# nauful/NLZM

Measured on AMD Instinct MI355X. Metric: compress MB/s, higher is better.
Workload: dtype u8; 1 GPU; enwik9 stand-in: 1000000000 B stream, -window:28; step = 41 launches of 8 chunks (40136704 B) of the stream; timed: bytes [200683520, 401367040) of 1000000000 (a prefix: the steps asked for end before the stream does); window_bits=28, batch_chunks=8, whole_stream=False

## Files before the change

nlzm_amd/csrc/nlzm_kernels.hip:

```cpp
#include <hip/hip_runtime.h>
#include <type_traits>
#include <cstddef>
#include <stdint.h>

#include "nlzm_core.h"
#include "nlzm_v2.h"

namespace nlzm {

#ifndef NLZM_LPW
#define NLZM_LPW 64
#endif
#ifndef NLZM_AHEAD
#define NLZM_AHEAD 3
#endif
constexpr uint32_t kAhead = NLZM_AHEAD;
constexpr uint32_t kEntryWords = 16;
union V2Lds {
    v2::FLds f; v2::TLds t; v2::PLds p;
    uint32_t wq[512 * kAhead * kEntryWords];
};
__shared__ V2Lds g_v2_lds;
}
namespace xw {
// ... 51 lines not shown
    for (int k = 0; k < 4; k++) {
        const uint32_t o = threadIdx.x + 256u * k;
        const unsigned long long a = blk0 + o;
        if (a >= a1) continue;
        uint32_t h = 0, h2 = 0;
        const bool ok = a + kPfLen <= n;
        if (ok) {
#pragma unroll 13
            for (uint32_t j = 0; j < kPfLen; j++) { h = (h + tile[o + j]) * 0x2F0FD693u; h2 = (h2 ^ tile[o + j]) * 0x01000193u + 0x7F4A7C15u; }
        }
        hbuf[a - a0] = h; hbuf2[a - a0] = h2;
        uint8_t f = 0;
        if (ok) {
            const unsigned long long sl = pf_slot(h, h2, t_bits);
            if (t_bitmap) f = (T[sl >> 5] >> (sl & 31u)) & 1u;
            else { const uint32_t t = T[sl]; f = t != 0 && (uint32_t)a - (t - 1) <= wmask; }
            atomicMin(&M[(h * kPfMul2) >> (32 - m_bits)], (uint32_t)a);
        }
        c1[a - a0] = f;
    }
}

__global__ __launch_bounds__(256) void prefilter_mark_kernel(unsigned long long n, uint32_t a0, uint32_t a1, uint32_t m_bits,
                                                             const uint32_t *__restrict__ M, const uint32_t *__restrict__ hbuf,
                                                             const uint8_t *__restrict__ c1, uint8_t *__restrict__ unc)
{
    const unsigned long long a = (unsigned long long)a0 + (unsigned long long)blockIdx.x * 256 + threadIdx.x;
    if (a >= a1) return;
    if (a == a0) unc[0] = 1;
    uint8_t f = c1[a - a0];
    if (a + kPfLen <= n) {
        const uint32_t h = hbuf[a - a0];
        f |= M[(h * kPfMul2) >> (32 - m_bits)] < (uint32_t)a;
    }
    if (a + 1 < a1) unc[a + 1 - a0] = f;
}

__global__ __launch_bounds__(256) void prefilter_insert_kernel(unsigned long long n, uint32_t a0, uint32_t a1, uint32_t t_bits, uint32_t t_bitmap,
                                                               uint32_t m_bits, uint32_t *__restrict__ T,
                                                               uint32_t *__restrict__ M, const uint32_t *__restrict__ hbuf,
                                                               const uint32_t *__restrict__ hbuf2)
{
    const unsigned long long a = (unsigned long long)a0 + (unsigned long long)blockIdx.x * 256 + threadIdx.x;
    if (a >= a1 || a + kPfLen > n) return;
    const uint32_t h = hbuf[a - a0];
    const unsigned long long sl = pf_slot(h, hbuf2[a - a0], t_bits);
    if (t_bitmap) atomicOr(&T[sl >> 5], 1u << (sl & 31u));
    else atomicMax(&T[sl], (uint32_t)a + 1);
    M[(h * kPfMul2) >> (32 - m_bits)] = kNone;
}

__global__ __launch_bounds__(1024) void bin_kernel(const uint8_t *__restrict__ in, Geom g, uint32_t c0,
                                                   uint32_t nheads , uint32_t *__restrict__ off_all,
                                                   uint32_t *__restrict__ cur_all, uint32_t *__restrict__ pos_all,
                                                   const uint8_t *__restrict__ unc, uint32_t batch_a0, uint32_t lds_bins)
{
    const uint32_t ci = c0 + blockIdx.x;
    uint32_t *off = off_all + (unsigned long long)blockIdx.x * (nheads + 1);
    uint32_t *cur = cur_all + (unsigned long long)blockIdx.x * nheads;
    uint32_t *pos = pos_all + (unsigned long long)blockIdx.x * g.chunk_size * 2;
    const unsigned long long chunk_abs = (unsigned long long)ci * g.chunk_size;
    const unsigned long long remain = g.n - chunk_abs;
    const uint32_t chunk_read = (uint32_t)(remain < g.feed ? remain : g.feed);
    const uint32_t p_end = umin(g.chunk_size, chunk_read);
    const uint32_t n_ok = chunk_read >= 4 ? umin(p_end, chunk_read - 3) : 0;
    const uint8_t *base = in + chunk_abs;
    __shared__ uint32_t part[1024];
    __shared__ uint32_t heads_t[1024];

    for (uint32_t p = threadIdx.x; p < n_ok; p += 1024) atomicAdd(&off[(hash4(load32u(base + p)) >> g.bt_shift) % nheads], 1u);
    __syncthreads();
    const uint32_t per = (nheads + 1023) / 1024;
    const uint32_t lo = umin(nheads, threadIdx.x * per), hi = umin(nheads, lo + per);
    uint32_t sum = 0;
    for (uint32_t h = lo; h < hi; h++) sum += off[h];
    part[threadIdx.x] = sum;
    __syncthreads();
    if (threadIdx.x == 0) {
        uint32_t run = 0;
        for (uint32_t t = 0; t < 1024; t++) { const uint32_t v = part[t]; part[t] = run; run += v; }
        off[nheads] = run;
    }
    __syncthreads();
    uint32_t run = part[threadIdx.x];
    for (uint32_t h = lo; h < hi; h++) { const uint32_t v = off[h]; off[h] = run; cur[h] = run; run += v; }
    __syncthreads();
    extern __shared__ uint32_t lcur[];
    if (nheads <= lds_bins) {
        for (uint32_t h = threadIdx.x; h < nheads; h += 1024) lcur[h] = off[h];
        __syncthreads();
        const uint32_t lane = threadIdx.x & 63u, wave = threadIdx.x >> 6;
        for (uint32_t t0 = 0; t0 < n_ok; t0 += 1024) {
            const uint32_t p = t0 + threadIdx.x;
            const bool ok = p < n_ok;
            const uint32_t hfull = ok ? hash4(load32u(base + p)) >> g.bt_shift : 0u;
            const uint32_t h = ok ? hfull % nheads : kNone;
            uint32_t rank = 0, cnt = 0, lead = lane;
            for (unsigned long long todo = __ballot(ok); todo;) {
                const uint32_t l = (uint32_t)__builtin_ctzll(todo);
                const uint32_t v = (uint32_t)__builtin_amdgcn_readlane((int)h, (int)l);
                const unsigned long long m = __ballot(ok && h == v);
                if (ok && h == v) { rank = (uint32_t)__builtin_popcountll(m & ((1ull << lane) - 1ull)); cnt = (uint32_t)__builtin_popcountll(m); lead = l; }
                todo &= ~m;
            }
            uint32_t first = 0;
            for (uint32_t w = 0; w < 16; w++) {
                if (wave == w && ok && lead == lane) { first = lcur[h]; lcur[h] = first + cnt; }
                __syncthreads();
            }
            first = (uint32_t)__shfl((int)first, (int)lead, 64);
            if (ok) {
                const uint32_t at = first + rank;
                const uint32_t a = (uint32_t)chunk_abs + p;
                pos[2 * at] = a;
                pos[2 * at + 1] = hfull | (unc[a - batch_a0] ? 0x80000000u : 0u) | ((a > batch_a0 && unc[a - batch_a0 - 1]) ? 0x40000000u : 0u) | (unc[a - batch_a0 + 1] ? 0x20000000u : 0u);
            }
        }
        return;
    }
    for (uint32_t t0 = 0; t0 < n_ok; t0 += 1024) {
        const uint32_t p = t0 + threadIdx.x;
        const bool ok = p < n_ok;
        const uint32_t hfull = ok ? hash4(load32u(base + p)) >> g.bt_shift : 0u;
        const uint32_t h = ok ? hfull % nheads : kNone;
        heads_t[threadIdx.x] = h;
        __syncthreads();
        uint32_t at = 0, after = 1;
        if (ok) {
            uint32_t before = 0;
            after = 0;
            for (uint32_t t = 0; t < 1024; t++) {
                const uint32_t o = heads_t[t];
                before += (o == h) & (t < threadIdx.x);
                after += (o == h) & (t > threadIdx.x);
            }
            at = cur[h] + before;
            const uint32_t a = (uint32_t)chunk_abs + p;
            pos[2 * at] = a;
            pos[2 * at + 1] = hfull | (unc[a - batch_a0] ? 0x80000000u : 0u) | ((a > batch_a0 && unc[a - batch_a0 - 1]) ? 0x40000000u : 0u) | (unc[a - batch_a0 + 1] ? 0x20000000u : 0u);
        }
        __syncthreads();
        if (ok && !after) cur[h] = at + 1;
        __syncthreads();
    }
}

__global__ __launch_bounds__(1024) void hot_select_kernel(const uint32_t *__restrict__ off_all, uint32_t nchunks, uint32_t nheads,
                                                          uint32_t hmax, uint32_t min_count, uint32_t *__restrict__ hot_of_bin,
                                                          uint32_t *__restrict__ hot_list, WorkerCounters *__restrict__ wcnt)
{
    __shared__ uint32_t hist[32];
    __shared__ uint32_t thr_s, n_s;
    if (threadIdx.x < 32) hist[threadIdx.x] = 0;
    if (threadIdx.x == 0) n_s = 0;
    __syncthreads();
    for (uint32_t b = threadIdx.x; b < nheads; b += 1024) {
        uint32_t tot = 0;
        for (uint32_t c = 0; c < nchunks; c++) {
            const uint32_t *off = off_all + (unsigned long long)c * (nheads + 1);
            tot += off[b + 1] - off[b];
        }
        hot_of_bin[b] = tot;
        if (tot >= min_count && tot) atomicAdd(&hist[31 - __builtin_clz(tot)], 1u);
    }
    __syncthreads();
    if (threadIdx.x == 0) {
        uint32_t acc = 0, k = 32;
        for (int j = 31; j >= 0; j--) {
            if (acc + hist[j] > hmax) break;
            acc += hist[j]; k = (uint32_t)j;
        }
        thr_s = k >= 32 ? 0xFFFFFFFFu : umax(min_count, 1u << k);
    }
    __syncthreads();
    const uint32_t thr = thr_s;
    for (uint32_t b = threadIdx.x; b < nheads; b += 1024) {
        const uint32_t tot = hot_of_bin[b];
        uint32_t v = 0;
        if (tot >= thr) {
            const uint32_t idx = atomicAdd(&n_s, 1u);
            if (idx < hmax) { hot_list[1 + idx] = b; v = idx + 1; }
        }
        hot_of_bin[b] = v;
    }
    __syncthreads();
    if (threadIdx.x == 0) { hot_list[0] = umin(n_s, hmax); atomicAdd(&wcnt->hot_bins, (unsigned long long)umin(n_s, hmax)); }
}

struct LaneIO {
    static __device__ __forceinline__ void st_agent(uint32_t *p, uint32_t v)
    {
        __hip_atomic_store(p, v, __ATOMIC_RELAXED, __HIP_MEMORY_SCOPE_AGENT);
    }
    static __device__ __forceinline__ uint32_t ld_agent(const uint32_t *p)
    {
        return __hip_atomic_load(p, __ATOMIC_RELAXED, __HIP_MEMORY_SCOPE_AGENT);
    }
    static __device__ __forceinline__ uint32_t atomic_inc(uint32_t *p) { return __hip_atomic_fetch_add(p, 1u, __ATOMIC_RELAXED, __HIP_MEMORY_SCOPE_AGENT); }
    static __device__ __forceinline__ void drain() { asm volatile("s_waitcnt vmcnt(0)" ::: "memory"); }
    static __device__ __forceinline__ void st_quad(uint32_t *p, uint32_t a, uint32_t b, uint32_t c, uint32_t d)
    {
        typedef uint32_t u4 __attribute__((ext_vector_type(4)));
        const u4 v = { a, b, c, d };
        asm volatile("global_store_dwordx4 %0, %1, off sc1\n\ts_nop 1" :: "v"((__attribute__((address_space(1))) uint32_t *)p), "v"(v) : "memory");
    }
};

struct LaneSink {
    uint32_t *slot;
    uint32_t *pairs;
    uint32_t count = 0, best = 1, best_d = 0;
    uint32_t ext_idx = 0;
    __device__ __forceinline__ void put(const BtView &B, uint32_t d, uint32_t l)
    {
        best = l; best_d = d;
        if (count < 4) { slot[(2 * count) * 512] = d; slot[(2 * count + 1) * 512] = l; }
        else {
            uint32_t *q = bt_pair_ptr<LaneIO>(pairs, B.pstride, B.ext, B.ext_cur, B.ext_cap, ext_idx, count);
            if (q) { LaneIO::st_agent(q, d); LaneIO::st_agent(q + 1, l); }
        }
        count++;
    }
    __device__ __forceinline__ void publish(uint32_t *rec, uint32_t tests) const
    {
        if (count > 4) LaneIO::drain();
        const uint32_t d0 = count > 0 ? slot[0] : 0u, l0 = count > 0 ? slot[512] : 0u, d1 = count > 1 ? slot[2 * 512] : 0u, l1 = count > 1 ? slot[3 * 512] : 0u;
        const uint32_t d2 = count > 2 ? slot[4 * 512] : 0u, l2 = count > 2 ? slot[5 * 512] : 0u, d3 = count > 3 ? slot[6 * 512] : 0u, l3 = count > 3 ? slot[7 * 512] : 0u;
        LaneIO::st_quad(rec + 4, d0, l0, d1, kBtTag);
        LaneIO::st_quad(rec + 8, l1, d2, l2, kBtTag);
        LaneIO::st_quad(rec + 12, d3, l3, ext_idx, kBtTag);
        LaneIO::st_quad(rec, kBtReady | (tests << 9) | count, best_d, count ? best : 0u, 0u);
    }
};
constexpr uint32_t kUndoCap = 260;
__device__ __forceinline__ void bt_descent(const BtView &B, uint32_t a, uint32_t hidx, uint32_t max_len, bool keep, bool dry, uint32_t *undo,
                                           uint32_t &n_undo, LaneSink &sink, uint32_t &tests_out, uint32_t &cmp_out)
{
    const uint8_t *pa = B.in + a;
    uint32_t sp = B.heads[hidx];
    uint32_t nu = 0;
    if (keep) { *(unsigned long long *)undo = (0x80000000u | hidx) | ((unsigned long long)(dry ? a : sp) << 32); nu = 1; }
    if (!dry) B.heads[hidx] = a;
    uint32_t pend_l = (a & B.tmask) << 1, pend_r = pend_l + 1, len_l = 0, len_r = 0, tests = 0, cb = 0;
    uint32_t old_l = kNone, old_r = kNone;
    while (sp != kNone && a > sp && a - sp <= B.wmask && tests < 256) {
        tests++;
        const uint32_t pair = (sp & B.tmask) << 1;
        const uint8_t *ps = B.in + sp;
        const uint32_t init = umin(len_l, len_r);
        const unsigned long long pp = *(const unsigned long long *)(B.tree + pair);
        const unsigned long long x0 = load64u(ps + init), y0 = load64u(pa + init), d0 = x0 ^ y0;
        const unsigned long long x1 = load64u(ps + init + 8), y1 = load64u(pa + init + 8), d1 = x1 ^ y1;
        const uint32_t nb0 = d0 ? (uint32_t)__builtin_ctzll(d0) >> 3 : (d1 ? 8u + ((uint32_t)__builtin_ctzll(d1) >> 3) : 16u);
        uint32_t l = init + nb0;
        bool full = l >= max_len;
        const unsigned long long xs = nb0 < 8 ? x0 : x1, ys = nb0 < 8 ? y0 : y1;
        uint32_t sign = (uint32_t)(((xs >> (8 * (nb0 & 7u))) & 0xFF) < ((ys >> (8 * (nb0 & 7u))) & 0xFF));
        if (nb0 == 16 && !full) {
            for (;;) {
                const unsigned long long x = load64u(ps + l), y = load64u(pa + l), d = x ^ y;
                if (d) {
                    const uint32_t nb = (uint32_t)__builtin_ctzll(d) >> 3;
                    l += nb;
                    sign = (uint32_t)(((x >> (8 * nb)) & 0xFF) < ((y >> (8 * nb)) & 0xFF));
                    break;
                }
                l += 8;
                if (l >= max_len) break;
            }
            full = l >= max_len;
        }
        if (full) l = max_len;
        cb += (l - init) + (full ? 0u : 1u);
        const uint32_t pl = (uint32_t)pp, pr = (uint32_t)(pp >> 32), d = a - sp;
        if (l >= match_min(d) && l > sink.best) sink.put(B, d, l);
        if (full) {
            if (!dry) { B.tree[pend_l] = pl; B.tree[pend_r] = pr; }
            if (keep) {
                *(unsigned long long *)(undo + 2 * nu) = pend_l | ((unsigned long long)(dry ? pl : old_l) << 32);
                *(unsigned long long *)(undo + 2 * nu + 2) = pend_r | ((unsigned long long)(dry ? pr : old_r) << 32);
                nu += 2;
            }
            tests_out = tests; cmp_out = cb; n_undo = nu;
            return;
        }
        const bool right = sign != 0;
        const uint32_t slot = right ? pend_l : pend_r;
        if (!dry) B.tree[slot] = sp;
        if (keep) { *(unsigned long long *)(undo + 2 * nu) = slot | ((unsigned long long)(dry ? sp : (right ? old_l : old_r)) << 32); nu++; }
        pend_l = right ? pair + 1 : pend_l; pend_r = right ? pend_r : pair;
        old_l = right ? pr : old_l; old_r = right ? old_r : pl;
        len_r = right ? l : len_r; len_l = right ? len_l : l;
        sp = right ? pr : pl;
    }
    if (!dry) { B.tree[pend_r] = kNone; B.tree[pend_l] = kNone; }
    if (keep) {
        *(unsigned long long *)(undo + 2 * nu) = pend_r | ((unsigned long long)(dry ? kNone : old_r) << 32);
        *(unsigned long long *)(undo + 2 * nu + 2) = pend_l | ((unsigned long long)(dry ? kNone : old_l) << 32);
        nu += 2;
    }
    tests_out = tests; cmp_out = cb; n_undo = nu;
}

#ifndef NLZM_RISKY_AHEAD
#define NLZM_RISKY_AHEAD 0
#endif
constexpr uint32_t kPending = 0xFFFFFFFEu;
__device__ __forceinline__ uint32_t wave_max_u32(uint32_t v) { return (uint32_t)__builtin_amdgcn_readlane((int)xw::scan_max(v), 63); }
__device__ __forceinline__ void worker_role_hot(const Geom &g, const Globals &G, uint32_t c0, uint32_t c1, uint32_t bin, uint32_t hot_index)
{
    unsigned long long p0 = (unsigned long long)G.in, p1 = (unsigned long long)G.bt_heads, p2 = (unsigned long long)G.bt_tree,
                       p3 = (unsigned long long)G.bt_ready, p4 = (unsigned long long)G.bt_pairs, p5 = (unsigned long long)G.bt_flag,
                       p6 = (unsigned long long)G.hot_undo;
    uint32_t q0 = G.batch_a0, q2 = g.wmask, q3 = g.bt_tmask;
    asm volatile("" : "+s"(p0), "+s"(p1), "+s"(p2), "+s"(p3), "+s"(p4), "+s"(p5), "+s"(p6));
    asm volatile("" : "+s"(q0), "+s"(q2), "+s"(q3));
#define NLZM_AS_GLOBAL(T, x) ((T *)(__attribute__((address_space(1))) T *)(x))
    const uint8_t *in = NLZM_AS_GLOBAL(const uint8_t, p0);
    uint32_t *heads = NLZM_AS_GLOBAL(uint32_t, p1), *tree = NLZM_AS_GLOBAL(uint32_t, p2), *ready = NLZM_AS_GLOBAL(uint32_t, p3);
    uint32_t *pairs = NLZM_AS_GLOBAL(uint32_t, p4);
    const uint32_t *flags = NLZM_AS_GLOBAL(const uint32_t, p5);
    const uint32_t lane = threadIdx.x & 63u;
    unsigned long long *const undo = NLZM_AS_GLOBAL(unsigned long long, p6) + ((unsigned long long)hot_index * 64 + lane) * kUndoCap;
#undef NLZM_AS_GLOBAL
    const uint32_t batch_a0 = q0, wmask = q2, tmask = q3;
    BtView Bx{ in, heads, tree, ready, pairs, batch_a0, 0u, wmask, tmask };
    Bx.pstride = G.bt_pstride; Bx.ext = G.bt_ext; Bx.ext_cur = G.bt_ext_cur; Bx.ext_cap = G.bt_ext_cap; Bx.fail_word = G.abort_word;
    enum : uint32_t { kIdle = 0, kStart = 1, kRun = 2, kHeld = 3 };
    enum : uint32_t { kwNone = 0, kwDone = 1, kwPark = 2, kwCall = 3 };
    uint32_t c = c0, wb = 0, cur = 0, e0 = 0, la_end = 0;
    const uint32_t *pos = G.bin_pos;
    bool loaded = false, more = true, wvalid = false, rec = false;
    unsigned long long w_pe = 0;
    uint32_t w_kind = kwNone;
    bool w_risky = false, w_wrong = false;
    unsigned long long o_pe = 0;
    bool o_park = false, o_risky = false, o_wrong = false, ovalid = false;
    uint32_t ob = 0;
    uint32_t st = kIdle, a = 0, hidx = 0, max_len = 0, sp = kNone, pend_l = 0, pend_r = 0, len_l = 0, len_r = 0, tests = 0, cb = 0;
    uint32_t seq = 0, nu = 0;
    uint32_t cmp_off = 0;
    bool marked = false, und = false, published = false, wrong = false;
    bool last_skip = false;
    LaneSink sink{ (uint32_t *)&g_v2_lds + threadIdx.x, nullptr };
    unsigned long long n_tests = 0, n_cmp = 0;
    uint32_t n_calls = 0, n_open = 0, n_back = 0, n_redo = 0;
    uint32_t n_steps = 0, n_blk_risky = 0;
    unsigned long long t_wait0 = 0;
    uint32_t prog_seen = 0, steps = 0;
    uint32_t k_work = 0, k_tests = 0, k_rep = 0, k_rec = 0, k_full = 0, k_blk = 0, k_noent = 0, k_skip = 0, k_und = 0;
    const unsigned long long k_t0 = __builtin_readcyclecounter();
    uint32_t k_total = 0;
    for (uint32_t cc = c0; cc < c1; cc++) { const uint32_t *off = G.bin_off + (unsigned long long)(cc - c0) * (G.nheads + 1); k_total += off[bin + 1] - off[bin]; }
#ifdef NLZM_PROFILE
    unsigned long long t_sec[7] = {}, t_last = __builtin_readcyclecounter();
#define NLZM_HOT_STAMP(k) do { const unsigned long long t_now = __builtin_readcyclecounter(); t_sec[k] += t_now - t_last; t_last = t_now; } while (0)
#else
#define NLZM_HOT_STAMP(k) do { } while (0)
#endif

    for (;;) {
        if (ovalid && !__any(o_park)) ovalid = false;
        if (wvalid && !ovalid && !rec && cur >= wb + umin(64u, e0 - wb) && cur < e0) {
            o_pe = w_pe; o_park = w_kind == kwPark; o_risky = w_risky; o_wrong = w_wrong; ob = wb; ovalid = true;
            wvalid = false; w_kind = kwNone; w_wrong = false; w_risky = false;
        }
        if (!wvalid && more && !rec) {
            for (;;) {
                if (!loaded) {
                    if (c >= c1) { more = false; break; }
                    const uint32_t *off = G.bin_off + (unsigned long long)(c - c0) * (G.nheads + 1);
                    cur = (uint32_t)__builtin_amdgcn_readfirstlane((int)off[bin]); e0 = (uint32_t)__builtin_amdgcn_readfirstlane((int)off[bin + 1]);
                    const unsigned long long chunk_abs = (unsigned long long)c * g.chunk_size;
                    const unsigned long long remain = g.n - chunk_abs;
                    la_end = (uint32_t)(chunk_abs + (remain < g.feed ? remain : g.feed));
                    pos = G.bin_pos + (unsigned long long)(c - c0) * g.chunk_size * 2;
                    loaded = true;
                }
                if (cur < e0) break;
                if (__any(st != kIdle) || ovalid) break;
                c++; loaded = false;
            }
            if (more && loaded && cur < e0) {
                wb = cur;
                const uint32_t idx = wb + lane;
                w_pe = 0; w_kind = kwNone; w_risky = false; w_wrong = false;
                if (idx < e0) {
                    w_pe = *(const unsigned long long *)(pos + 2 * idx);
                    const bool mk = (w_pe >> 63) != 0;
                    uint32_t f = 0;
                    if (mk) f = LaneIO::ld_agent(flags + ((uint32_t)w_pe - batch_a0));
                    w_kind = !mk ? kwCall : (f == kFlagSkip ? kwDone : (f == kFlagCall ? kwCall : ((w_pe >> 61) == 7u ? kwPark : kwCall)));
                    k_skip += mk && f == kFlagSkip;
                }
                wvalid = true;
            }
        }
        NLZM_HOT_STAMP(6);
        const uint32_t wend = wvalid ? umin(64u, e0 - wb) : 0u;
        const bool w_und = wvalid && w_kind == kwPark && wb + lane < cur;
        const bool o_und = ovalid && o_park;
        const uint32_t w_seq = wb + lane + 1, o_seq = ob + lane + 1;
        const unsigned long long w_um = __ballot(w_und), o_um = __ballot(o_und);
        uint32_t oseq = 0xFFFFFFFFu, rseq = 0xFFFFFFFFu;
        if (__any(und)) oseq = ~wave_max_u32(und ? ~seq : 0u);
        if (w_um) oseq = umin(oseq, wb + (uint32_t)__builtin_ctzll(w_um) + 1u);
        if (o_um) oseq = umin(oseq, ob + (uint32_t)__builtin_ctzll(o_um) + 1u);
        if (__any(wrong || w_wrong || (ovalid && o_wrong))) {
            rseq = ~wave_max_u32(umax(wrong ? ~seq : 0u, umax(w_wrong ? ~w_seq : 0u, (ovalid && o_wrong) ? ~o_seq : 0u)));
            rec = true;
        }
        if (rec && !__any(st == kStart || st == kRun)) {
            for (;;) {
                const uint32_t smax = wave_max_u32(st == kHeld && seq > rseq ? seq : 0u);
                if (!smax) break;
                if (st == kHeld && seq == smax) {
                    for (uint32_t j = nu; j-- > 0;) {
                        const unsigned long long w = undo[j];
                        const uint32_t t = (uint32_t)w, v = (uint32_t)(w >> 32);
                        if (t >> 31) heads[t & 0x7FFFFFFFu] = v; else tree[t] = v;
                    }
                    st = kIdle; und = false; wrong = false; n_redo++;
                }
            }
            if (st == kHeld && seq == rseq) {
                for (uint32_t j = nu; j-- > 0;) {
                    const unsigned long long w = undo[j];
                    const uint32_t t = (uint32_t)w, v = (uint32_t)(w >> 32);
                    if (t >> 31) heads[t & 0x7FFFFFFFu] = v; else tree[t] = v;
                }
                st = kIdle; und = false; wrong = false; n_back++;
            }
            const bool parked = __any((w_wrong && w_seq == rseq) || (ovalid && o_wrong && o_seq == rseq));
            if (parked && lane == 0) n_back++;
            cur = parked ? rseq - 1 : rseq;
            if (ovalid && cur < ob + 64) {
                if (cur >= ob) {
                    w_pe = o_pe; w_kind = o_park ? kwPark : kwDone; w_risky = o_risky; w_wrong = o_wrong; wb = ob; wvalid = true;
                } else wvalid = false;
                ovalid = false; o_park = false; o_wrong = false;
            } else if (wvalid && cur < wb) wvalid = false;
            if (wvalid) {
                const uint32_t idx = wb + lane;
                if (idx >= cur) {
                    w_kind = kwNone; w_risky = false; w_wrong = false;
                    if (idx < e0) {
                        w_pe = *(const unsigned long long *)(pos + 2 * idx);
                        const bool mk = (w_pe >> 63) != 0;
                        uint32_t f = 0;
                        if (mk) f = LaneIO::ld_agent(flags + ((uint32_t)w_pe - batch_a0));
                        w_kind = !mk ? kwCall : (f == kFlagSkip ? kwDone : (f == kFlagCall ? kwCall : ((w_pe >> 61) == 7u ? kwPark : kwCall)));
                    }
                }
            } else { w_wrong = false; w_kind = kwNone; }
            rec = false;
            continue;
        }
        NLZM_HOT_STAMP(0);
        uint32_t start_lane = 64;
        unsigned long long pe = 0;
        uint32_t pe_seq = 0;
        bool made_test = false, rep_step = false, started_now = false;
        const unsigned long long free_m = __ballot(st == kIdle);
        const bool risky_open = __any((w_und && w_risky) || (o_und && o_risky));
        bool call_blocked = false;
        n_steps++;
        if (wvalid && !rec && cur < wb + wend) {
            const uint32_t cl = cur - wb;
            const unsigned long long range = (~0ull << cl) & (wend < 64 ? (1ull << wend) - 1ull : ~0ull);
            const unsigned long long mC = __ballot(w_kind == kwCall) & range, mP = __ballot(w_kind == kwPark) & range;
            const uint32_t c1i = mC ? (uint32_t)__builtin_ctzll(mC) : 64u, p1 = mP ? (uint32_t)__builtin_ctzll(mP) : 64u;
            bool call_ok = c1i < 64 && free_m && !risky_open && !(!last_skip && p1 < c1i);
            call_blocked = c1i < 64 && free_m && !call_ok;
            uint32_t end = cl;
            if (!risky_open) {
                end = c1i;
                if (call_ok) {
                    const unsigned long long restC = mC & ~(1ull << c1i);
                    end = restC ? (uint32_t)__builtin_ctzll(restC) : 64u;
                }
                if (!last_skip && p1 < end) end = p1 + 1;
            }
            if (call_ok) {
                start_lane = (uint32_t)__builtin_ctzll(free_m);
                pe = ((unsigned long long)(uint32_t)__builtin_amdgcn_readlane((int)(uint32_t)(w_pe >> 32), (int)c1i) << 32) | (uint32_t)__builtin_amdgcn_readlane((int)(uint32_t)w_pe, (int)c1i);
                pe_seq = wb + c1i + 1;
            }
            end = umin(end, wend);
            if (w_kind == kwPark && lane >= cl && lane < end) w_risky = !last_skip;
            if (call_ok && lane == c1i) w_kind = kwDone;
            cur = wb + end;
        }
        if (call_blocked) n_blk_risky++;
        if (lane == start_lane) {
            a = (uint32_t)pe; hidx = (uint32_t)(pe >> 32) & 0x1FFFFFFFu;
            max_len = umin(la_end - a, kMatchMax);
            marked = (pe >> 63) != 0;
            seq = pe_seq;
            st = kStart;
        }
        if (wvalid && cur >= wb + wend && !__any(w_kind == kwPark)) wvalid = false;
        NLZM_HOT_STAMP(1);
        uint32_t v_word = 0, v_flag = 0, w_flag = 0;
        unsigned long long pp = 0, x0 = 0, y0 = 0, x1 = 0, y1 = 0;
        bool fin_now = false;
        uint32_t fin_l = kNone, fin_r = kNone;
        if (st == kRun && !(sp != kNone && a > sp && a - sp <= wmask && tests < 256)) fin_now = true;
        const uint32_t pair = (sp & tmask) << 1, init = umin(len_l, len_r);
        if ((st == kStart && marked) || und) v_flag = LaneIO::ld_agent(flags + (a - batch_a0));
        uint32_t o_flag = 0;
        {
            const unsigned long long om = __ballot(o_und && !o_wrong), wm = __ballot(w_und && !w_wrong);
            const uint32_t o_rank = __builtin_amdgcn_mbcnt_hi((uint32_t)(om >> 32), __builtin_amdgcn_mbcnt_lo((uint32_t)om, 0u));
            const uint32_t w_rank = __builtin_amdgcn_mbcnt_hi((uint32_t)(wm >> 32), __builtin_amdgcn_mbcnt_lo((uint32_t)wm, 0u)) + (uint32_t)__builtin_popcountll(om);
            if (o_und && !o_wrong && o_rank < 8u) o_flag = LaneIO::ld_agent(flags + ((uint32_t)o_pe - batch_a0));
            if (w_und && !w_wrong && w_rank < 8u) w_flag = LaneIO::ld_agent(flags + ((uint32_t)w_pe - batch_a0));
        }
        if (st == kStart) v_word = heads[hidx];
        else if (st == kRun && !fin_now) {
            pp = *(const unsigned long long *)(tree + pair);
            const uint8_t *ps = in + sp + init + cmp_off, *pa = in + a + init + cmp_off;
            x0 = load64u(ps); y0 = load64u(pa); x1 = load64u(ps + 8); y1 = load64u(pa + 8);
        }
        {
            const bool decided = und && !wrong && (v_flag == kFlagCall || v_flag == kFlagSkip);
            if (decided) {
                if (v_flag == kFlagCall) und = false;
                else wrong = true;
            }
            const bool w_decided = w_und && !w_wrong && (w_flag == kFlagCall || w_flag == kFlagSkip);
            if (w_decided) {
                if (w_flag == kFlagSkip) w_kind = kwDone;
                else w_wrong = true;
            }
            const bool o_decided = o_und && !o_wrong && (o_flag == kFlagCall || o_flag == kFlagSkip);
            if (o_decided) {
                if (o_flag == kFlagSkip) o_park = false;
                else o_wrong = true;
            }
            if (__any(decided || w_decided || o_decided))
                last_skip = __any((decided && v_flag == kFlagSkip) || (w_decided && w_flag == kFlagSkip) || (o_decided && o_flag == kFlagSkip));
        }
#ifdef NLZM_PROFILE
        asm volatile("s_waitcnt vmcnt(0)" ::: "memory");
#endif
        NLZM_HOT_STAMP(2);
        if (st == kStart) {
            bool go = true;
            if (marked) {
                if (v_flag == kFlagSkip) { st = kIdle; go = false; }
                else if (v_flag != kFlagCall) { und = true; n_open++; }
            }
            if (go) {
                started_now = true;
                sp = v_word;
                pend_l = (a & tmask) << 1; pend_r = pend_l + 1; len_l = 0; len_r = 0; tests = 0; cb = 0; cmp_off = 0;
                sink.count = 0; sink.best = 1; sink.best_d = 0; sink.ext_idx = 0; sink.pairs = pairs + (unsigned long long)(a - batch_a0) * (2 * Bx.pstride);
                published = false;
                undo[0] = (0x80000000u | hidx) | ((unsigned long long)sp << 32);
                nu = 1;
                *(unsigned long long *)(tree + pend_l) = ((unsigned long long)kPending << 32) | kPending;
                heads[hidx] = a;
                st = kRun;
            }
        } else if (st == kRun && !fin_now) {
            const unsigned long long d0 = x0 ^ y0, d1 = x1 ^ y1;
            const uint32_t from = init + cmp_off;
            uint32_t nb = d0 ? (uint32_t)__builtin_ctzll(d0) >> 3 : (d1 ? 8u + ((uint32_t)__builtin_ctzll(d1) >> 3) : 16u);
            uint32_t l = from + nb;
            bool full = l >= max_len;
            const unsigned long long xs = nb < 8 ? x0 : x1, ys = nb < 8 ? y0 : y1;
            const uint32_t sign = (uint32_t)(((xs >> (8 * (nb & 7u))) & 0xFF) < ((ys >> (8 * (nb & 7u))) & 0xFF));
            const uint32_t pl = (uint32_t)pp, pr = (uint32_t)(pp >> 32);
            const bool more_cmp = nb == 16 && !full;
            if (more_cmp) cmp_off += 16;
            if (full) l = max_len;
            const bool right = sign != 0;
            const bool held = more_cmp || (full ? (pl == kPending || pr == kPending) : ((right ? pr : pl) == kPending));
            rep_step = held;
            if (!held) {
                made_test = true;
                cmp_off = 0;
                tests++;
                cb += (l - init) + (full ? 0u : 1u);
                const uint32_t d = a - sp;
                if (l >= match_min(d) && l > sink.best) sink.put(Bx, d, l);
                if (full) { fin_now = true; fin_l = pl; fin_r = pr; }
                else {
                    const uint32_t slot = right ? pend_l : pend_r;
                    tree[right ? pair + 1 : pair] = kPending;
                    asm volatile("" ::: "memory");
                    tree[slot] = sp;
                    asm volatile("" ::: "memory");
                    undo[nu] = (right ? pair + 1 : pair) | ((unsigned long long)(right ? pr : pl) << 32);
                    nu++;
                    pend_l = right ? pair + 1 : pend_l; pend_r = right ? pend_r : pair;
                    len_r = right ? l : len_r; len_l = right ? len_l : l;
                    sp = right ? pr : pl;
                }
            }
        }
        NLZM_HOT_STAMP(3);
        if (fin_now) {
            tree[pend_l] = fin_l; tree[pend_r] = fin_r;
            st = kHeld;
        }
        if (st == kHeld && !wrong) {
            if (!published && seq <= oseq) { sink.publish(ready + (unsigned long long)(a - batch_a0) * kBtRec, tests); published = true; }
            if (published && !und && seq <= oseq) {
                n_calls++; n_tests += tests; n_cmp += cb;
                st = kIdle;
            }
        }
        NLZM_HOT_STAMP(4);
#ifdef NLZM_PROFILE
        {
            const uint32_t nt = (uint32_t)__builtin_popcountll(__ballot(made_test)), nr = (uint32_t)__builtin_popcountll(__ballot(rep_step));
            k_tests += nt; k_rep += nr;
            if (nt || __any(started_now)) k_work++;
            else {
                if (rec) k_rec++;
                else if (!free_m) k_full++;
                else if (call_blocked) k_blk++;
                else k_noent++;
                if (__any(und || w_und || o_und)) k_und++;
            }
        }
#else
        (void)made_test; (void)rep_step; (void)started_now;
#endif
        if ((++steps & 4095u) == 0) {
            if (__any(LaneIO::ld_agent(G.abort_word) != 0)) break;
            if (__any(und || w_und || o_und)) {
                const unsigned long long now = wall_clock64();
                const uint32_t prog = G.progress ? (uint32_t)__builtin_amdgcn_readfirstlane((int)LaneIO::ld_agent(G.progress)) : 0u;
                if (!t_wait0 || prog != prog_seen) { t_wait0 = now; prog_seen = prog; }
                else if (now - t_wait0 > 3000000000ull) { if (lane == 0) LaneIO::st_agent(G.abort_word, 2u); break; }
            } else t_wait0 = 0;
        }
        NLZM_HOT_STAMP(5);
        if (!more && !wvalid && !ovalid && !rec && !__any(st != kIdle)) break;
    }
    if (st != kIdle) {
        atomicAdd(&G.wcnt->stuck_lanes, 1ull);
        atomicMax(&G.wcnt->stuck_pos_inv, (unsigned long long)(uint32_t)~a);
    }
    unsigned long long t_calls = n_calls, t_open = n_open, t_back = n_back, t_redo = n_redo, t_skip = k_skip;
    for (int m = 32; m >= 1; m >>= 1) {
        t_calls += __shfl_xor(t_calls, m, 64); n_tests += __shfl_xor(n_tests, m, 64); n_cmp += __shfl_xor(n_cmp, m, 64);
        t_open += __shfl_xor(t_open, m, 64); t_back += __shfl_xor(t_back, m, 64); t_redo += __shfl_xor(t_redo, m, 64);
        t_skip += __shfl_xor(t_skip, m, 64);
    }
    if (lane == 0) {
        atomicAdd(&G.wcnt->bt_calls, t_calls); atomicAdd(&G.wcnt->bt_tests, n_tests); atomicAdd(&G.wcnt->cmp_bytes, n_cmp);
        atomicAdd(&G.wcnt->dry_runs, t_open); atomicAdd(&G.wcnt->spec_calls, t_back); atomicAdd(&G.wcnt->spec_good, t_redo);
        atomicAdd(&G.wcnt->hot_calls, t_calls);
        atomicAdd(&G.wcnt->hot_steps, (unsigned long long)n_steps); atomicAdd(&G.wcnt->hot_blocked_risky, (unsigned long long)n_blk_risky);
        uint32_t kc = 0;
        while (kc < 7 && (k_total >> (14 + kc))) kc++;
        unsigned long long *hc = G.wcnt->hot_class[kc];
        atomicAdd(&hc[kHcWaves], 1ull); atomicAdd(&hc[kHcCalls], t_calls); atomicAdd(&hc[kHcTests], n_tests); atomicAdd(&hc[kHcSteps], (unsigned long long)n_steps); atomicAdd(&hc[kHcTestSteps], (unsigned long long)k_work);
        atomicAdd(&hc[kHcLaneTests], (unsigned long long)k_tests); atomicAdd(&hc[kHcRepeats], (unsigned long long)k_rep); atomicAdd(&hc[kHcTakingBack], (unsigned long long)k_rec); atomicAdd(&hc[kHcAllHold], (unsigned long long)k_full); atomicAdd(&hc[kHcMayNotStart], (unsigned long long)k_blk);
        atomicAdd(&hc[kHcNoEntry], (unsigned long long)k_noent); atomicAdd(&hc[kHcCycles], (unsigned long long)(__builtin_readcyclecounter() - k_t0)); atomicAdd(&hc[kHcSkipped], t_skip); atomicAdd(&hc[kHcIdleUndecided], (unsigned long long)k_und);
#ifdef NLZM_PROFILE
        for (uint32_t z = 0; z < kHcSecN; z++) atomicAdd(&hc[kHcSec + z], t_sec[z]);
#endif
    }
#undef NLZM_HOT_STAMP
}

__device__ __forceinline__ void worker_role(const Geom &g, const Globals &G, uint32_t c0, uint32_t c1, uint32_t wblocks, uint32_t wblock)
{
    constexpr uint32_t kLpw = NLZM_LPW;
    const uint32_t lane_waves = (G.wthreads + kLpw - 1) / kLpw;
    if ((threadIdx.x >> 6) >= lane_waves) {
        if (!G.hot_list) return;
        const uint32_t k = ((threadIdx.x >> 6) - lane_waves) * wblocks + wblock;
        if (k >= G.hot_list[0]) return;
        worker_role_hot(g, G, c0, c1, G.hot_list[1 + k], k);
        return;
    }
    const uint32_t lane_in_block = (threadIdx.x >> 6) * kLpw + (threadIdx.x & 63u);
    const bool takes_bin = (threadIdx.x & 63u) < kLpw && lane_in_block < G.wthreads;
    const uint32_t gl = wblock * G.wthreads + (takes_bin ? lane_in_block : 0u);
    unsigned long long p0 = (unsigned long long)G.in, p1 = (unsigned long long)G.bt_heads, p2 = (unsigned long long)G.bt_tree,
                       p3 = (unsigned long long)G.bt_ready, p4 = (unsigned long long)G.bt_pairs;
    uint32_t q0 = G.batch_a0, q1 = g.bt_shift, q2 = g.wmask, q3 = g.bt_tmask;
    asm volatile("" : "+s"(p0), "+s"(p1), "+s"(p2), "+s"(p3), "+s"(p4));
    asm volatile("" : "+s"(q0), "+s"(q1), "+s"(q2), "+s"(q3));
#define NLZM_AS_GLOBAL(T, x) ((T *)(__attribute__((address_space(1))) T *)(x))
    BtView B{ NLZM_AS_GLOBAL(const uint8_t, p0), NLZM_AS_GLOBAL(uint32_t, p1), NLZM_AS_GLOBAL(uint32_t, p2), NLZM_AS_GLOBAL(uint32_t, p3),
              NLZM_AS_GLOBAL(uint32_t, p4), q0, q1, q2, q3 };
    B.pstride = G.bt_pstride; B.ext = G.bt_ext; B.ext_cur = G.bt_ext_cur; B.ext_cap = G.bt_ext_cap; B.fail_word = G.abort_word;
    uint32_t *const undo_base = NLZM_AS_GLOBAL(uint32_t, (unsigned long long)G.bt_undo) + (unsigned long long)gl * (kAhead * kUndoCap * 2);
#undef NLZM_AS_GLOBAL
    bool active = takes_bin && gl < G.nheads && !(G.hot_of_bin && G.hot_of_bin[gl < G.nheads ? gl : 0]);
    uint32_t c = c0;
    bool loaded = false;
    uint32_t i0 = 0, e0 = 0;
    uint32_t la_end = 0;
    unsigned long long n_calls = 0, n_tests = 0, n_cmp = 0, n_open = 0, n_wait = 0, n_cyc = 0, n_cyc_tests = 0, n_back = 0, n_redo = 0;
    uint32_t first = 0, nq = 0, head_a = 0;
    uint32_t *const my = (uint32_t *)&g_v2_lds + threadIdx.x;
    enum : uint32_t { kWa = 8, kWtests = 9, kWcmp = 10, kWcount = 11, kWbest = 12, kWbestd = 13, kWundo = 14, kWinfo = 15 };
    unsigned long long t_wait0 = 0;
    uint32_t idle = 0, prog_seen = 0;
    bool fail = false;

    while (__any(active)) {
        bool waiting = false;
        uint32_t job = 0, ja = 0, jh = 0, jlen = 0, jinfo = 0;
        if (active) {
            if (nq) {
                const uint32_t f = LaneIO::ld_agent(G.bt_flag + (head_a - G.batch_a0));
                const bool hdry = (my[(first * kEntryWords + kWinfo) * 512] >> 28) & 1u;
                if ((f == kFlagCall && !hdry) || (f == kFlagSkip && hdry)) {
                    for (uint32_t k = 0; k < kAhead; k++) {
                        uint32_t *e = my + (first * kEntryWords) * 512;
                        if (!((e[kWinfo * 512] >> 28) & 1u)) { n_calls++; n_tests += e[kWtests * 512]; n_cmp += e[kWcmp * 512]; }
                        first = first + 1 == kAhead ? 0u : first + 1; nq--;
                        if (!nq) break;
                        e = my + (first * kEntryWords) * 512;
                        const uint32_t ea = e[kWa * 512], einfo = e[kWinfo * 512];
                        if (!((einfo >> 28) & 1u)) {
                            LaneSink sk{ e, B.pairs + (unsigned long long)(ea - B.batch_a0) * (2 * B.pstride), e[kWcount * 512] & 0x1FFu, e[kWbest * 512], e[kWbestd * 512], e[kWcount * 512] >> 9 };
                            sk.publish(B.ready + (unsigned long long)(ea - B.batch_a0) * kBtRec, e[kWtests * 512]);
                        }
                        if (einfo & 1u) {
                            head_a = ea;
                            const uint32_t f2 = LaneIO::ld_agent(G.bt_flag + (ea - G.batch_a0));
                            const bool edry = (einfo >> 28) & 1u;
                            if (!((f2 == kFlagCall && !edry) || (f2 == kFlagSkip && edry))) break;
                        }
                    }
                } else if (f == kFlagCall || f == kFlagSkip) {
                    uint32_t resume = i0;
                    for (uint32_t k = nq; k-- > 0;) {
                        const uint32_t slot = first + k >= kAhead ? first + k - kAhead : first + k;
                        const uint32_t *e = my + (slot * kEntryWords) * 512;
                        const uint32_t *u = undo_base + slot * (kUndoCap * 2);
                        if (k == 0 || !((e[kWinfo * 512] >> 28) & 1u)) {
                            for (uint32_t j = e[kWundo * 512]; j-- > 0;) {
                                const unsigned long long w = *(const unsigned long long *)(u + 2 * j);
                                const uint32_t t = (uint32_t)w, v = (uint32_t)(w >> 32);
                                if (t >> 31) B.heads[t & 0x7FFFFFFFu] = v; else B.tree[t] = v;
                            }
                        }
                        if (k == 1) resume = (e[kWinfo * 512] & 0xFFFFFFu) >> 1;
                        if (k == 0 && hdry) resume = (e[kWinfo * 512] & 0xFFFFFFu) >> 1;
                        if (k) n_redo++;
                    }
                    n_back++;
                    i0 = resume; nq = 0;
                }
            }
            if (nq < kAhead) {
                if (!loaded) {
                    if (c >= c1) { if (!nq) active = false; }
                    else {
                        const uint32_t *off = G.bin_off + (unsigned long long)(c - c0) * (G.nheads + 1);
                        i0 = off[gl]; e0 = off[gl + 1];
                        const unsigned long long chunk_abs = (unsigned long long)c * g.chunk_size;
                        const unsigned long long remain = g.n - chunk_abs;
                        la_end = (uint32_t)(chunk_abs + (remain < g.feed ? remain : g.feed));
                        loaded = true;
                    }
                }
                if (active && loaded) {
                    const uint32_t *pos = G.bin_pos + (unsigned long long)(c - c0) * g.chunk_size * 2;
                    if (i0 >= e0) { if (!nq) { c++; loaded = false; } }
                    else {
                        const unsigned long long pe = *(const unsigned long long *)(pos + 2 * i0);
                        ja = (uint32_t)pe; jh = (uint32_t)(pe >> 32) & 0x1FFFFFFFu; jlen = umin(la_end - ja, kMatchMax);
                        jinfo = (i0 << 1) | (uint32_t)(pe >> 63);
                        i0++;
                        if (pe >> 63) {
                            const uint32_t f = LaneIO::ld_agent(G.bt_flag + (ja - G.batch_a0));
                            job = f == kFlagSkip ? 0u : ((f == kFlagCall && !nq) ? 1u : 2u);
#ifdef NLZM_EXP_SKIP_ANY
                            if (f != kFlagCall && ((pe >> 61) & 3u) != 0u) jinfo |= 1u << 28;
#else
                            if (f != kFlagCall && ((pe >> 61) & 3u) == 3u) jinfo |= 1u << 28;
#endif
                        } else job = nq ? 2u : 1u;
                    }
                }
            }
            if (!job && nq) {
                waiting = true;
                n_wait++;
                if ((++idle & 1023u) == 0) {
                    if (LaneIO::ld_agent(G.abort_word)) active = false;
                    const unsigned long long now = wall_clock64();
                    const uint32_t prog = G.progress ? LaneIO::ld_agent(G.progress) : 0u;
                    if (!t_wait0 || prog != prog_seen) { t_wait0 = now; prog_seen = prog; }
                    else if (now - t_wait0 > 3000000000ull) { fail = true; }
                }
            }
            if (fail) { LaneIO::st_agent(G.abort_word, 2u); active = false; job = 0; }
        }
        if (job) {
            const unsigned long long t0 = __builtin_readcyclecounter();
            const unsigned long long bi = ja - B.batch_a0;
            const uint32_t slot = first + nq >= kAhead ? first + nq - kAhead : first + nq;
            uint32_t *e = my + (slot * kEntryWords) * 512;
            LaneSink sink{ e, B.pairs + bi * (2 * B.pstride) };
            uint32_t tests = 0, cmpb = 0, nu = 0;
            const bool park = job == 2 && ((jinfo >> 28) & 1u);
            if (!park) bt_descent(B, ja, jh, jlen, job == 2, false, undo_base + slot * (kUndoCap * 2), nu, sink, tests, cmpb);
            if (job == 1) {
                sink.publish(B.ready + bi * kBtRec, tests);
                n_calls++; n_tests += tests; n_cmp += cmpb;
                n_cyc += __builtin_readcyclecounter() - t0; n_cyc_tests += tests;
            } else {
                if (!nq) { if (!park) sink.publish(B.ready + bi * kBtRec, tests); head_a = ja; t_wait0 = 0; idle = 0; }
                e[kWa * 512] = ja; e[kWtests * 512] = tests; e[kWcmp * 512] = cmpb; e[kWcount * 512] = sink.count | (sink.ext_idx << 9);
                e[kWbest * 512] = sink.best; e[kWbestd * 512] = sink.best_d; e[kWundo * 512] = nu; e[kWinfo * 512] = jinfo;
                nq++; if (!park) n_open++;
            }
        }
        if (!__any(active && !waiting)) __builtin_amdgcn_s_sleep(8);
    }
    if (nq) {
        atomicAdd(&G.wcnt->stuck_lanes, 1ull);
        atomicMax(&G.wcnt->stuck_pos_inv, (unsigned long long)(uint32_t)~head_a);
    }
    for (int m = 32; m >= 1; m >>= 1) {
        n_calls += __shfl_xor(n_calls, m, 64); n_tests += __shfl_xor(n_tests, m, 64); n_cmp += __shfl_xor(n_cmp, m, 64);
        n_open += __shfl_xor(n_open, m, 64); n_wait += __shfl_xor(n_wait, m, 64);
        n_cyc += __shfl_xor(n_cyc, m, 64); n_cyc_tests += __shfl_xor(n_cyc_tests, m, 64);
        n_back += __shfl_xor(n_back, m, 64); n_redo += __shfl_xor(n_redo, m, 64);
    }
    if ((threadIdx.x & 63) == 0) {
        atomicAdd(&G.wcnt->bt_calls, n_calls); atomicAdd(&G.wcnt->bt_tests, n_tests); atomicAdd(&G.wcnt->cmp_bytes, n_cmp);
        atomicAdd(&G.wcnt->dry_runs, n_open); atomicAdd(&G.wcnt->flag_waits, n_wait);
        atomicAdd(&G.wcnt->call_cycles, n_cyc); atomicAdd(&G.wcnt->call_tests, n_cyc_tests);
        atomicAdd(&G.wcnt->spec_calls, n_back); atomicAdd(&G.wcnt->spec_good, n_redo);
    }
}

constexpr uint32_t kV2Roles = 3 + v2::kHelpers;
__device__ __forceinline__ void pipeline2_roles(const Geom &g, const Globals &G, const v2::GlobalsV2 &V, uint32_t c0, uint32_t c1,
                                                uint32_t local_block, uint32_t wblocks)
{
    if (local_block < kV2Roles) {
        if (threadIdx.x >= (local_block >= 2 ? v2::kParserThreads : (local_block == 1 ? 64u * v2::table_waves(((const v2::StateV2 *)V.state)->tb_wide[G.launch_par & 1u]) : 64u))) return;
        if (local_block == 0) { v2::Finder r; r.g = g; r.G = G; r.V = V; r.run(c0, c1); }
        else if (local_block == 1) { v2::Table r; r.g = g; r.G = G; r.V = V; r.run(c0, c1); }
        else if (local_block == 2) { v2::Parser r; r.g = g; r.G = G; r.V = V; r.run(c0, c1); }
        else if (V.hb) { v2::Parser r; r.g = g; r.G = G; r.V = V; r.run_helper(c0, local_block - 3); }
    } else {
        worker_role(g, G, c0, c1, wblocks, local_block - kV2Roles);
    }
}
__global__ __launch_bounds__(512) void pipeline2_kernel(Geom g, Globals G, v2::GlobalsV2 V, uint32_t c0, uint32_t c1)
{
    const uint32_t b = blockIdx.x;
    const bool spread = gridDim.x > 8 * (kV2Roles - 1);
    const uint32_t before = b ? (b + 7) / 8 < kV2Roles ? (b + 7) / 8 : kV2Roles : 0u;
    const uint32_t local = (b % 8 == 0 && b / 8 < kV2Roles && spread) ? b / 8 : (spread ? kV2Roles + (b - before) : b);
    pipeline2_roles(g, G, V, c0, c1, local, gridDim.x - kV2Roles);
}
struct Stream2Args { Geom g; Globals G; v2::GlobalsV2 V; uint32_t c0, c1; v2::RoundSnap *snap; };
constexpr uint32_t kMaxStreams2PerLaunch = 64;
__global__ __launch_bounds__(512) void pipeline2_multi_kernel(const Stream2Args *__restrict__ pack, uint32_t bps)
{
    uint32_t s, local;
    multi_block_of(gridDim.x, bps, blockIdx.x, s, local);
    Stream2Args a = pack[s];
#define NLZM_GLOBAL_PTR(p) p = (decltype(p))(__attribute__((address_space(1))) std::remove_pointer_t<decltype(p)> *)(unsigned long long)(p)
    NLZM_GLOBAL_PTR(a.G.in); NLZM_GLOBAL_PTR(a.G.rkhash); NLZM_GLOBAL_PTR(a.G.ht2); NLZM_GLOBAL_PTR(a.G.ht3); NLZM_GLOBAL_PTR(a.G.rk_table);
    NLZM_GLOBAL_PTR(a.G.bt_heads); NLZM_GLOBAL_PTR(a.G.bt_tree); NLZM_GLOBAL_PTR(a.G.persist); NLZM_GLOBAL_PTR(a.G.syms); NLZM_GLOBAL_PTR(a.G.bits);
    NLZM_GLOBAL_PTR(a.G.fmeta); NLZM_GLOBAL_PTR(a.G.cap_words); NLZM_GLOBAL_PTR(a.G.cap_used); NLZM_GLOBAL_PTR(a.G.bt_ready); NLZM_GLOBAL_PTR(a.G.bt_pairs); NLZM_GLOBAL_PTR(a.G.bt_ext); NLZM_GLOBAL_PTR(a.G.bt_ext_cur);
    NLZM_GLOBAL_PTR(a.G.bt_flag); NLZM_GLOBAL_PTR(a.G.unc); NLZM_GLOBAL_PTR(a.G.bin_off); NLZM_GLOBAL_PTR(a.G.bin_pos); NLZM_GLOBAL_PTR(a.G.abort_word);
    NLZM_GLOBAL_PTR(a.G.progress); NLZM_GLOBAL_PTR(a.G.wcnt); NLZM_GLOBAL_PTR(a.G.bt_undo); NLZM_GLOBAL_PTR(a.G.hot_of_bin); NLZM_GLOBAL_PTR(a.G.hot_list); NLZM_GLOBAL_PTR(a.G.hot_undo);
    NLZM_GLOBAL_PTR(a.V.ft); NLZM_GLOBAL_PTR(a.V.tp); NLZM_GLOBAL_PTR(a.V.tf); NLZM_GLOBAL_PTR(a.V.hx); NLZM_GLOBAL_PTR(a.V.state); NLZM_GLOBAL_PTR(a.V.hb);
#undef NLZM_GLOBAL_PTR
    pipeline2_roles(a.g, a.G, a.V, a.c0, a.c1, local, bps - kV2Roles);
}
#define NLZM_G(T, x) ((__attribute__((address_space(1))) T *)(unsigned long long)(x))
__global__ __launch_bounds__(256) void round_open_kernel(const Stream2Args *__restrict__ pack)
{
    const Stream2Args &a = pack[blockIdx.x];
    auto *w = NLZM_G(uint32_t, a.V.hx);
    const uint32_t a0 = a.G.batch_a0;
    constexpr uint32_t kWords = sizeof(v2::Hx) / 4;
    const uint32_t sticky = NLZM_G(const uint32_t, a.G.persist)[offsetof(Persist, error) / 4];
    for (uint32_t i = threadIdx.x; i < kWords; i += 256) {
        uint32_t v = 0;
        if (i == offsetof(v2::Hx, f_pos) / 4 || i == offsetof(v2::Hx, t_pos) / 4 || i == offsetof(v2::Hx, t_out) / 4 || i == offsetof(v2::Hx, p_pos) / 4 ||
            i == offsetof(v2::Hx, p_seg) / 4 || i == offsetof(v2::Hx, p_seg) / 4 + 1) v = a0;
        if (i == offsetof(v2::Hx, err) / 4) v = sticky;
        w[i] = v;
    }
    if (threadIdx.x == 0 && sticky && a.G.abort_word) *NLZM_G(uint32_t, a.G.abort_word) = 1u;
}
__global__ __launch_bounds__(256) void round_close_kernel(const Stream2Args *__restrict__ pack)
{
    const Stream2Args &a = pack[blockIdx.x];
    const auto *w = NLZM_G(const uint32_t, a.V.hx);
    auto *o = NLZM_G(uint32_t, a.snap);
    constexpr uint32_t kHead = offsetof(v2::RoundSnap, hx) / 4;
    for (uint32_t i = threadIdx.x; i < sizeof(v2::Hx) / 4; i += 256) o[kHead + i] = w[i];
    if (threadIdx.x == 0) {
        const auto *ps = NLZM_G(const uint32_t, a.G.persist);
        o[0] = ps[offsetof(Persist, error) / 4]; o[1] = ps[offsetof(Persist, next_chunk) / 4];
        o[2] = a.G.abort_word ? *NLZM_G(const uint32_t, a.G.abort_word) : 0u; o[3] = 0;
    }
}
#undef NLZM_G

__global__ __launch_bounds__(256) void rans_frames_kernel(const uint32_t *__restrict__ syms, unsigned long long syms_stride,
                                                          const uint8_t *__restrict__ bits, unsigned long long bits_stride,
                                                          FrameMeta *__restrict__ fmeta, uint32_t *__restrict__ scratch,
                                                          unsigned long long scratch_stride,
                                                          uint8_t *__restrict__ out, unsigned long long out_stride,
                                                          uint32_t out_cap)
{
    const uint32_t f = blockIdx.x;
    const uint32_t n = fmeta[f].nsyms, nb = fmeta[f].nbits_bytes, ops = fmeta[f].num_ops;
    const uint32_t *s = syms + f * syms_stride;
    uint32_t *w = scratch + f * scratch_stride;
    uint8_t *o = out + f * out_stride;
    __shared__ uint32_t st_final[4];
    __shared__ uint32_t wave_tot[4];
    __shared__ uint32_t carry_s;

    if (threadIdx.x < 4) {
        uint32_t x = 1u << 16;
        const uint32_t k = threadIdx.x;
        if (n > k) {
            for (long long i = (long long)(((n - 1 - k) & ~3u) + k); i >= 0; i -= 4) {
                const uint32_t v = s[i];
                const uint32_t start = v & 0xFFFFu, freq = v >> 16;
                uint32_t pushed = kNone;
                if (x >= (freq << 18)) {
                    pushed = x & 0xFFFFu;
                    x >>= 16;
                }
                w[i] = pushed;
                x = ((x / freq) << 14) + (x % freq) + start;
            }
        }
        st_final[k] = x;
    }
    if (threadIdx.x == 0) carry_s = 0;
    __syncthreads();

    const uint32_t lane = threadIdx.x & 63, wv = threadIdx.x >> 6;
    for (uint32_t i = threadIdx.x; i < nb; i += 256) if (12 + i < out_cap) o[12 + i] = bits[f * bits_stride + i];
    uint8_t *r = o + 12 + nb;
    if (threadIdx.x < 16 && 12 + nb + 16 <= out_cap) {
        const uint32_t x = st_final[threadIdx.x >> 2];
        r[threadIdx.x] = (uint8_t)(x >> (8 * (threadIdx.x & 3)));
    }
    for (uint32_t base = 0; base < n; base += 256) {
        const uint32_t i = base + threadIdx.x;
        const uint32_t word = i < n ? w[i] : kNone;
        const bool has = word != kNone;
        const unsigned long long bal = __ballot(has);
        const uint32_t before = (uint32_t)__popcll(bal & ((1ull << lane) - 1));
        if (lane == 0) wave_tot[wv] = (uint32_t)__popcll(bal);
        __syncthreads();
        uint32_t off = carry_s;
        for (uint32_t k = 0; k < wv; k++) off += wave_tot[k];
        if (has) {
            const uint32_t at = 12 + nb + 16 + 2 * (off + before);
            if (at + 2 <= out_cap) { o[at] = (uint8_t)(word >> 8); o[at + 1] = (uint8_t)word; }
        }
        __syncthreads();
        if (threadIdx.x == 0) carry_s += wave_tot[0] + wave_tot[1] + wave_tot[2] + wave_tot[3];
        __syncthreads();
    }
    if (threadIdx.x == 0) {
        const uint32_t nrans = 16 + 2 * carry_s;
        const uint32_t hdr[3] = { ops, 12 + nb, nrans };
        for (int k = 0; k < 3; k++) {
            o[4 * k + 0] = (uint8_t)(hdr[k] >> 24); o[4 * k + 1] = (uint8_t)(hdr[k] >> 16);
            o[4 * k + 2] = (uint8_t)(hdr[k] >> 8);  o[4 * k + 3] = (uint8_t)hdr[k];
        }
        fmeta[f].out_len = 12 + nb + nrans;
    }
}

__global__ __launch_bounds__(256) void gather_frames_kernel(const uint8_t *__restrict__ frames, unsigned long long stride,
                                                            const unsigned long long *__restrict__ dst_off,
                                                            const FrameMeta *__restrict__ fmeta, uint8_t *__restrict__ dst)
{
    const uint32_t f = blockIdx.x;
    const uint32_t len = fmeta[f].out_len;
    const uint8_t *s = frames + f * stride;
    uint8_t *d = dst + dst_off[f];
    for (uint32_t i = threadIdx.x; i < len; i += 256) d[i] = s[i];
}

void launch_rk_hash(const uint8_t *in, unsigned long long n, unsigned long long pos0, unsigned long long pos1,
                    uint32_t *out, hipStream_t st)
{
    if (pos1 <= pos0) return;
    const unsigned long long blocks = (pos1 - pos0 + 1023) / 1024;
    hipLaunchKernelGGL(rk_hash_kernel, dim3((uint32_t)blocks), dim3(256), 0, st, in, n, pos0, pos1, out);
}

void launch_pipeline2(const Geom &g, const Globals &G, const v2::GlobalsV2 &V, uint32_t c0, uint32_t c1, uint32_t worker_blocks, hipStream_t st)
{
    hipLaunchKernelGGL(pipeline2_kernel, dim3(kV2Roles + worker_blocks), dim3(512), 0, st, g, G, V, c0, c1);
}
unsigned long long stream2_pack_size() { return sizeof(Stream2Args) * kMaxStreams2PerLaunch; }
uint32_t stream2_pack_capacity() { return kMaxStreams2PerLaunch; }
uint32_t pipeline2_role_blocks() { return kV2Roles; }
void fill_stream2_args(void *host_pack, uint32_t i, const Geom &g, const Globals &G, const v2::GlobalsV2 &V, uint32_t c0, uint32_t c1, v2::RoundSnap *snap)
{
    Stream2Args &a = ((Stream2Args *)host_pack)[i];
    a.g = g; a.G = G; a.V = V; a.c0 = c0; a.c1 = c1; a.snap = snap;
}
void launch_round_open(const void *dev_pack, uint32_t nstreams, hipStream_t st)
{
    hipLaunchKernelGGL(round_open_kernel, dim3(nstreams), dim3(256), 0, st, (const Stream2Args *)dev_pack);
}
void launch_round_close(const void *dev_pack, uint32_t nstreams, hipStream_t st)
{
    hipLaunchKernelGGL(round_close_kernel, dim3(nstreams), dim3(256), 0, st, (const Stream2Args *)dev_pack);
}
void launch_pipeline2_multi(const void *dev_pack, uint32_t nstreams, uint32_t worker_blocks, hipStream_t st)
{
    hipLaunchKernelGGL(pipeline2_multi_kernel, dim3(nstreams * (kV2Roles + worker_blocks)), dim3(512), 0, st, (const Stream2Args *)dev_pack,
                       kV2Roles + worker_blocks);
}

void launch_prefilter(const uint8_t *in, unsigned long long n, uint32_t a0, uint32_t a1, uint32_t wmask, uint32_t t_bits, uint32_t t_bitmap,
                      uint32_t m_bits, uint32_t *T, uint32_t *M, uint32_t *hbuf, uint32_t *hbuf2, uint8_t *c1, uint8_t *unc, hipStream_t st)
{
    if (a1 <= a0) return;
    const uint32_t cnt = a1 - a0;
    hipLaunchKernelGGL(prefilter_hash_kernel, dim3((cnt + 1023) / 1024), dim3(256), 0, st, in, n, a0, a1, wmask, t_bits, t_bitmap, m_bits,
                       T, M, hbuf, hbuf2, c1);
    hipLaunchKernelGGL(prefilter_mark_kernel, dim3((cnt + 255) / 256), dim3(256), 0, st, n, a0, a1, m_bits, M, hbuf, c1, unc);
    hipLaunchKernelGGL(prefilter_insert_kernel, dim3((cnt + 255) / 256), dim3(256), 0, st, n, a0, a1, t_bits, t_bitmap, m_bits, T, M, hbuf, hbuf2);
}

void launch_bin(const uint8_t *in, const Geom &g, uint32_t c0, uint32_t nchunks, uint32_t nheads, uint32_t *off, uint32_t *cur,
                uint32_t *pos, const uint8_t *unc, uint32_t batch_a0, hipStream_t st)
{
    if (!nchunks) return;
    constexpr uint32_t kBinsInLdsMax = 36864;
    const uint32_t lds_bins = nheads <= kBinsInLdsMax ? nheads : 0u;
    (void)hipFuncSetAttribute((const void *)bin_kernel, hipFuncAttributeMaxDynamicSharedMemorySize, (int)(kBinsInLdsMax * 4));
    hipLaunchKernelGGL(bin_kernel, dim3(nchunks), dim3(1024), lds_bins * 4, st, in, g, c0, nheads, off, cur, pos, unc, batch_a0, lds_bins);
}

void launch_hot_select(const uint32_t *off, uint32_t nchunks, uint32_t nheads, uint32_t hmax, uint32_t min_count, uint32_t *hot_of_bin,
                       uint32_t *hot_list, WorkerCounters *wcnt, hipStream_t st)
{
    hipLaunchKernelGGL(hot_select_kernel, dim3(1), dim3(1024), 0, st, off, nchunks, nheads, hmax, min_count, hot_of_bin, hot_list, wcnt);
}

unsigned long long worker_hot_undo_bytes_per_wave() { return 64ull * kUndoCap * 8; }
unsigned long long worker_undo_bytes_per_lane() { return (unsigned long long)kAhead * kUndoCap * 8; }

void launch_rans(const uint32_t *syms, unsigned long long syms_stride, const uint8_t *bits, unsigned long long bits_stride,
                 FrameMeta *fmeta, uint32_t *scratch, unsigned long long scratch_stride, uint8_t *out,
                 unsigned long long out_stride, uint32_t out_cap, uint32_t nframes, hipStream_t st)
{
    if (!nframes) return;
    hipLaunchKernelGGL(rans_frames_kernel, dim3(nframes), dim3(256), 0, st, syms, syms_stride, bits, bits_stride, fmeta,
                       scratch, scratch_stride, out, out_stride, out_cap);
}

void launch_gather(const uint8_t *frames, unsigned long long stride, const unsigned long long *dst_off,
                   const FrameMeta *fmeta, uint8_t *dst, uint32_t nframes, hipStream_t st)
{
    if (!nframes) return;
    hipLaunchKernelGGL(gather_frames_kernel, dim3(nframes), dim3(256), 0, st, frames, stride, dst_off, fmeta, dst);
}

}
```

nlzm_amd/csrc/nlzm_v2.h:

```cpp
#pragma once

#include "nlzm_core.h"
#include "xw.h"

namespace nlzm {
namespace v2 {

constexpr uint32_t kFtRing = 1u << 14;
constexpr uint32_t kFtStride = 16;
constexpr uint32_t kTpRing = 1u << 13;
constexpr uint32_t kMaxEdges = 32;
constexpr uint32_t kTpStride = 2 + 2 + 2 * kMaxEdges;
constexpr uint32_t kTpUniq = 2, kTpEdges = 4;
constexpr uint32_t kFrontMax = 264;
constexpr uint32_t kTfStride = 2 * kFrontMax;

constexpr uint32_t kFtBt = 8u, kFtTop = 16u;
struct Hx {
    alignas(128) uint32_t f_pos;
    alignas(128) uint32_t t_pos;
    alignas(128) uint32_t t_out;
    alignas(128) uint32_t p_pos;
    alignas(128) unsigned long long p_seg;
    alignas(128) uint32_t h_job;
    struct alignas(128) HelpWords {
        alignas(128) uint32_t verdict;
        alignas(128) unsigned long long prog;
        alignas(128) uint32_t state;
    } hw[3];
    alignas(128) uint32_t ext_cur;
    alignas(128) uint32_t err;
    uint32_t err_info[7];
    alignas(128) uint32_t dbg[4][32];
};
enum : uint32_t { kStFinder = 11, kStTable = 12, kStParser = 13 };
enum DbgRow : uint32_t { kDbgFinder = 0, kDbgTable = 1, kDbgParser = 2 };
enum DbgFinderWord : uint32_t { kDfBlock, kDfReach, kDfTopActive, kDfTopDist, kDfTopEnd, kDfPrevNice, kDfSegStart, kDfRkLen, kDfTPosSeen, kDfErr, kDfBase, kDfWords };
enum DbgTableWord : uint32_t { kDtCursor, kDtTurn, kDtCarrySeq, kDtFSeen, kDtPSeen, kDtCarryN, kDtWords };
enum DbgParserWord : uint32_t { kDpChunk, kDpSegment, kDpBlockNode, kDpMaxParse, kDpStaged, kDpTOutSeen, kDpErr, kDpWords };
static_assert(kDfWords == 11 && kDtWords == 6 && kDpWords == 7, "Hx::dbg rows");
struct RoundSnap { uint32_t error, next_chunk, aborted, pad; Hx hx; };

#ifndef NLZM_HELPERS
#define NLZM_HELPERS 2
#endif
constexpr uint32_t kHelpers = NLZM_HELPERS;
static_assert(kHelpers >= 1 && kHelpers <= 3, "Hx::hw holds three helpers' words");
NLZM_HD uint32_t help_start(uint32_t k) { return kHelpers == 1 ? 1792u : (kHelpers == 2 ? (k == 0 ? 1280u : 2496u) : 880u * (k + 1)); }
constexpr uint32_t kHelpWarm = 576;
constexpr uint32_t kHelpExit = 0xFFFFFFFFu;
struct HelpBox {
    uint32_t seg_a, chunk_left, base, pad0, rep[4];
    alignas(16) uint16_t price[kNumCtx * 16];
    alignas(16) uint16_t len_price[kMatchMax + 8];
    alignas(16) uint16_t slot_price[4 * 64];
    alignas(16) uint32_t link[kParseMax + 2], delta[kParseMax + 2], cost[kParseMax + 2], rep_of[(kParseMax + 2) * 4], cmpw[4][kParseMax + 2];
    uint32_t seg_len, end_rep[4];
    alignas(16) uint32_t relist[512 * kTpStride];
};
constexpr unsigned long long kStagedOwn = 0x80000000ull;

struct GlobalsV2 {
    uint32_t *ft;
    uint32_t *tp;
    uint32_t *tf;
    Hx *hx;
    uint32_t *state;
    HelpBox *hb;
};

struct StateV2 {
    uint32_t reach, reach_d;
    uint32_t s_active, s_d, s_end, s_seen;
    uint32_t prev_nice, seg_s;
    uint32_t front_n;
    uint32_t front[2 * kFrontMax];
    uint32_t tb_wide[2];
};

constexpr uint32_t kErrV2Front = 40;
constexpr uint32_t kErrV2Promise = 41;
constexpr uint32_t kErrV2Edges = 42;

NLZM_HD uint32_t umin3(uint32_t a, uint32_t b, uint32_t c) { return umin(a, umin(b, c)); }

XW_FN uint32_t wave_cmp(const uint8_t *in, uint32_t s, uint32_t t, uint32_t init, uint32_t cap)
{
    uint32_t off = init;
    while (off < cap) {
        const uint32_t my = off + xw::lane() * 8;
        uint32_t m = kNone;
        if (my < cap) {
            const unsigned long long d = load64u(in + s + my) ^ load64u(in + t + my);
            if (d) {
                const uint32_t p = my + ((uint32_t)__builtin_ctzll(d) >> 3);
                if (p < cap) m = p;
            }
        }
        const unsigned long long bal = xw::ballot(m != kNone);
        if (bal) return xw::readlane(m, (uint32_t)__builtin_ctzll(bal));
        off += 512;
    }
    return cap;
}

XW_FN void raise(Hx *hx, uint32_t code, uint32_t stage, uint32_t site, uint32_t pos, uint32_t x0 = 0, uint32_t x1 = 0)
{
    if (xw::cas_agent(&hx->err, 0u, code) != 0u) return;
    xw::st_agent(&hx->err_info[0], stage); xw::st_agent(&hx->err_info[1], site); xw::st_agent(&hx->err_info[2], pos);
    xw::st_agent(&hx->err_info[3], x0); xw::st_agent(&hx->err_info[4], x1);
}

XW_FN bool wait_word_ge(const uint32_t *w, uint32_t v, Hx *hx, uint32_t code)
{
    if ((int32_t)(xw::readfirst(xw::ld_agent(w)) - v) >= 0) { xw::after_poll(); return true; }
    const unsigned long long t0 = xw::clock100();
    uint32_t spins = 0;
    for (;;) {
        if ((int32_t)(xw::readfirst(xw::ld_agent(w)) - v) >= 0) { xw::after_poll(); return true; }
        if ((++spins & 63u) == 0) {
            if (xw::readfirst(xw::ld_agent(&hx->err))) return false;
#ifndef NLZM_SIM
            if (xw::clock100() - t0 > 3000000000ull) {
                if (xw::lane() == 0) raise(hx, kErrTimeout * 100 + code, code == 1 ? kStFinder : (code <= 3 ? kStTable : kStParser), code, v, xw::ld_agent(w));
                return false;
            }
#else
            (void)t0; (void)code;
#endif
        }
        xw::pause();
    }
}

struct FLds {
    uint32_t ht2[4096];
    uint32_t ht3[16384 + 8];
    uint32_t stage[64 * kFtStride];
    uint32_t job[64 * 3 * 4];
    uint32_t job_len[64 * 4];
    uint32_t njobs;
    uint32_t last[8192];
    Counters cnt;
};

struct Finder {
    Geom g;
    Globals G;
    GlobalsV2 V;
    uint32_t base;
    uint32_t reach;
    uint32_t reach_d = kNone;
    uint32_t s_active, s_d, s_end, s_seen;
    uint32_t rk_from, rk_to, rk_len, rk_end;
    uint32_t rk_cut = 0;
    uint32_t prev_nice, seg_s;
    uint32_t gap_last = 0;
    uint32_t n_seg_own = 0, n_seg_wait = 0;
    uint32_t t_pos_seen;
    uint32_t err;
    uint32_t dbg_a = 0;
    unsigned long long n_pos, n_nice, n_unc, n_ht, n_rkp, n_rki, n_cmp, n_blocks, n_cut0, n_cut1, n_cut2, n_cut3, n_cut4, n_cut5;
    unsigned long long n_cmp_lane = 0;
    unsigned long long t_wait, t_wait_bt = 0, t_total;
    uint32_t n_so_top = 0, n_so_tie = 0, n_so_won = 0;
    uint32_t n_late_unc = 0, n_late_other = 0, n_late_hot = 0, n_late_first = 0, n_late_blocks = 0;
    unsigned long long t_f[kPfFinderSecN] = {};
#ifdef NLZM_PROFILE
    XW_FN unsigned long long ptick() const { return xw::tick(); }
#else
    XW_FN unsigned long long ptick() const { return 0; }
#endif

    XW_FN void fail(uint32_t code, uint32_t pos, uint32_t site = 0, uint32_t x0 = 0, uint32_t x1 = 0)
    {
        err = code;
        if (xw::lane() == 0) raise(V.hx, code, kStFinder, site, pos, x0, x1);
    }

    uint32_t pend_fpos = 0;
    uint32_t pf_a0 = kNone, pf_rkh = 0;
    unsigned long long pf_own0 = 0, pf_own1 = 0;
    uint8_t pf_unc = 0;
    XW_FN void flush_fpos()
    {
        if (!pend_fpos) return;
        xw::drain();
        if (xw::lane() == 0) xw::st_agent(&V.hx->f_pos, pend_fpos);
        pend_fpos = 0;
    }

    XW_FN void slider_look(uint32_t limit)
    {
        while (s_end == kNone && s_seen < limit) {
            const uint32_t cap = umin(limit - s_seen, 512u);
            const uint32_t l = wave_cmp(G.in, s_seen - s_d, s_seen, 0, cap);
            if (l < cap) s_end = s_seen + l; else s_seen += cap;
        }
        if (s_end == kNone && (unsigned long long)s_seen >= g.n) s_end = (uint32_t)g.n;
    }

    XW_FN uint32_t block(uint32_t a0, uint32_t n, uint32_t a1, uint32_t la_end)
    {
        FLds *L = xw::lds<FLds>();
        const uint32_t i = xw::lane();
        const bool in_blk = i < n;
        const uint32_t a = a0 + i, q = a - base;
        const uint32_t avail = in_blk ? la_end - a : 0u;
        const uint32_t cap = umin(avail, kMatchMax);
        const uint8_t *cur = G.in + a;
        const unsigned long long bi = (unsigned long long)(a - G.batch_a0);

        if (s_active) slider_look(umin(a0 + n + kMatchMax, la_end));
        const bool s_known = s_active && s_end != kNone;
        const uint32_t s_e = s_active ? (s_known ? umin(s_end, a + cap) : a + cap) : 0u;
        const bool s_sliding = s_active && (!s_known || s_end >= a + cap);
        const unsigned long long closed_mask = xw::ballot(in_blk && s_active && !s_sliding);
        const uint32_t jc = closed_mask ? (uint32_t)__builtin_ctzll(closed_mask) : 64u;

        const unsigned long long f0 = ptick();
        const uint32_t reach_pred = umax(reach, s_e);
        const bool nice_pred = in_blk && reach_pred >= a + kNice && reach_pred > a;
        if (xw::readlane(nice_pred ? 1u : 0u, 0) && !prev_nice) {
            if (a0 == (uint32_t)((unsigned long long)(a0 / g.chunk_size) * g.chunk_size)) seg_s = a0;
            else {
                flush_fpos();
                const unsigned long long tw = xw::tick();
                const unsigned long long t0 = xw::clock100();
                uint32_t spins = 0;
                for (;;) {
                    const unsigned long long ps = xw::readfirst64(xw::ld_agent64(&V.hx->p_seg));
                    const uint32_t sa = (uint32_t)(ps >> 32), cover = (uint32_t)ps;
                    const bool covered = (int32_t)(cover - (a0 + 1)) >= 0;
                    const bool own = !covered && (int32_t)(gap_last - cover) < 0 && a0 - sa < kParseMax;
                    if (covered || own) {
                        xw::after_poll();
                        seg_s = sa;
                        n_seg_own += own; n_seg_wait += spins != 0;
                        xw::trace(1, a0, seg_s, (uint32_t)ps);
                        break;
                    }
                    if ((++spins & 63u) == 0) {
                        if (xw::readfirst(xw::ld_agent(&V.hx->err))) { err = kErrInternal + 100; return 1; }
#ifndef NLZM_SIM
                        if (xw::clock100() - t0 > 3000000000ull) { fail(kErrTimeout, a0, 5, (uint32_t)ps, (uint32_t)(ps >> 32)); return 1; }
#else
                        (void)t0;
#endif
                    }
                    xw::pause();
                }
                t_wait += xw::tick() - tw;
            }
        }
        const bool call_full = in_blk && !nice_pred;
        const bool call_some = call_full || (nice_pred && ((a - seg_s) & 7u) == 0);
        const bool ht_call = call_some && avail >= 4;
        const bool rk_call = call_some && avail >= 256;

        uint32_t cut_rk = 64;
        {
            const unsigned long long rkm = xw::ballot(rk_call);
            if (rkm & 1ull) {
                const uint32_t q0 = a0 - base;
                for (uint32_t e = (rk_end | 255u) + 1; e < q0 + 256; e += 256) {
                    const uint32_t hh = xw::readfirst(G.rkhash[base + e - 256]);
                    if (i == 0) G.rk_table[hh >> g.rk_shift] = q0 | (hh << g.wbits);
                    n_rki++;
                }
                xw::drain();
            }
            const unsigned long long below = rkm & ((1ull << i) - 1);
            const uint32_t prev_end = below ? (a0 + (63u - (uint32_t)__builtin_clzll(below))) - base + 256 : rk_end;
            const bool catch_up = rk_call && i > 0 && ((prev_end | 255u) + 1) < q + 256;
            const unsigned long long cm = xw::ballot(catch_up);
            if (cm) cut_rk = (uint32_t)__builtin_ctzll(cm);
        }

        const unsigned long long f1 = ptick();
        uint32_t v4 = 0;
        unsigned long long own0 = 0, own1 = 0;
        uint32_t rkh = 0;
        bool unc = false;
        if (pf_a0 == a0) {
            if (in_blk) { own0 = pf_own0; own1 = pf_own1; v4 = (uint32_t)own0; }
            rkh = rk_call ? pf_rkh : 0u;
            unc = in_blk && G.workers && pf_unc != 0;
        } else {
            if (in_blk) { own0 = load64u(cur); own1 = load64u(cur + 8); v4 = (uint32_t)own0; }
            rkh = rk_call ? G.rkhash[a] : 0u;
            unc = in_blk && G.workers && G.unc[bi] != 0;
        }
        uint32_t rkv = rk_call ? G.rk_table[rkh >> g.rk_shift] : 0u;
        const bool bt_call = call_full && avail >= 4 && G.workers;

        const unsigned long long f2 = ptick();
        const uint32_t h2 = hash4(v4 & 0xFFFFu), h3 = hash4(v4 & 0xFFFFFFu);
        const uint32_t i2 = h2 >> 20, i3 = h3 >> g.ht3_shift;
        const uint32_t tag2 = h2 & g.tag_mask, tag3 = h3 & g.tag_mask;
        const uint32_t e2 = q | (tag2 << g.wbits), e3 = q | (tag3 << g.wbits);
        uint32_t row2 = 0, r0 = 0, r1 = 0;
        if (ht_call) { row2 = L->ht2[i2]; r0 = L->ht3[i3]; r1 = L->ht3[i3 + 1]; }
        const unsigned long long htm = xw::ballot(ht_call);
        bool later = false;
        {
            uint32_t *last = L->last;
            if (ht_call) { xw::lds_max(&last[i2], i + 1); xw::lds_max(&last[4096 + (i3 & 4095u)], i + 1); }
            xw::wave_sync();
            if (ht_call) later = last[i2] > i + 1 || last[4096 + (i3 & 4095u)] > i + 1 || last[4096 + ((i3 + 1) & 4095u)] > i + 1 || last[4096 + ((i3 - 1) & 4095u)] > i + 1;
            xw::wave_sync();
            if (ht_call) { last[i2] = 0; last[4096 + (i3 & 4095u)] = 0; }
        }
        const unsigned long long dep = xw::ballot(later);
        for (unsigned long long mm = dep; mm; mm &= mm - 1) {
            const uint32_t j = (uint32_t)__builtin_ctzll(mm);
            const uint32_t b2 = xw::readlane(i2, j), b3 = xw::readlane(i3, j);
            const uint32_t x2 = xw::readlane(e2, j), x3 = xw::readlane(e3, j), y0 = xw::readlane(r0, j);
            if (ht_call && i > j) {
                if (i2 == b2) row2 = x2;
                if (i3 == b3) { r0 = x3; r1 = y0; }
                else if (i3 == b3 + 1) r0 = y0;
                else if (i3 + 1 == b3) r1 = x3;
            }
        }

        const unsigned long long f3 = ptick();
        uint32_t cd[4] = { 0, 0, 0, 0 };
        if (ht_call) {
            const uint32_t s0 = row2 & g.wmask, s1 = r0 & g.wmask, s2 = r1 & g.wmask;
            if ((row2 >> g.wbits) == tag2 && s0 < q && q - s0 <= g.wmask) cd[0] = q - s0;
            if ((r0 >> g.wbits) == tag3 && s1 < q && q - s1 <= g.wmask) cd[1] = q - s1;
            if ((r1 >> g.wbits) == tag3 && s2 < q && q - s2 <= g.wmask) cd[2] = q - s2;
        }
        const bool rk_act = rk_len > 0 && q - rk_to < rk_len;
        const uint32_t rk_eff = rk_act ? rk_len : 0u;
        const bool rk_probe = rk_call && rk_eff < 256;
        bool rk_cand = false;
        uint32_t rk_d = 0;
        if (rk_probe) {
            const uint32_t sp = rkv & g.wmask;
            if ((rkv >> g.wbits) == (rkh & g.tag_mask) && sp < q && q - sp <= g.wmask) { rk_cand = true; rk_d = q - sp; }
        }
        uint32_t rk_l16 = 16;
        if (rk_cand) {
            const unsigned long long x0 = load64u(cur - rk_d) ^ own0;
            if (x0) rk_l16 = (uint32_t)__builtin_ctzll(x0) >> 3;
            else {
                const unsigned long long x1 = load64u(cur - rk_d + 8) ^ own1;
                rk_l16 = x1 ? 8 + ((uint32_t)__builtin_ctzll(x1) >> 3) : 16;
            }
        }
        const bool rk_short = rk_cand && rk_l16 < 16 && rk_l16 < (avail & 0xFFFFu);
        const bool rk_dropped = rk_short && !(rk_l16 >= rk_eff && rk_l16 >= match_min(rk_d));
        uint32_t cl[3] = { 0, 0, 0 };
        L->njobs = 0;
        xw::wave_sync();
        unsigned long long cx0[3], cx1[3];
#pragma unroll
        for (int k = 0; k < 3; k++) {
            cx0[k] = cd[k] ? load64u(cur - cd[k]) : 0ull;
            cx1[k] = cd[k] ? load64u(cur - cd[k] + 8) : 0ull;
        }
#pragma unroll
        for (int k = 0; k < 3; k++) {
            if (!cd[k]) continue;
            const unsigned long long x0 = cx0[k] ^ own0;
            uint32_t l;
            if (x0) l = (uint32_t)__builtin_ctzll(x0) >> 3;
            else {
                const unsigned long long x1 = cx1[k] ^ own1;
                l = x1 ? 8 + ((uint32_t)__builtin_ctzll(x1) >> 3) : 16;
            }
            if (l >= cap) l = cap;
            else if (l == 16) {
                const uint32_t at = xw::lds_inc(&L->njobs);
                L->job[at * 4] = i | ((uint32_t)k << 8); L->job[at * 4 + 1] = cd[k]; L->job[at * 4 + 2] = cap;
                l = kNone;
            }
            cl[k] = l;
        }
        xw::wave_sync();
        {
            const uint32_t nj = xw::readfirst(L->njobs);
            for (uint32_t jb = 0; jb < nj; jb += 8) {
                const uint32_t j = jb + (i >> 3), sub = i & 7u;
                const bool have = j < nj;
                const uint32_t jl = have ? L->job[j * 4] : 0u, jd = have ? L->job[j * 4 + 1] : 1u, jcap = have ? L->job[j * 4 + 2] : 0u;
                const uint32_t ja = a0 + (jl & 63u);
                uint32_t res = kNone;
                bool open = have;
                uint32_t off = 16;
                while (xw::any(open)) {
                    uint32_t pos = kNone;
                    const uint32_t my = off + sub * 8;
                    if (open && my < jcap) {
                        const unsigned long long d = load64u(G.in + ja - jd + my) ^ load64u(G.in + ja + my);
                        if (d) { const uint32_t p = my + ((uint32_t)__builtin_ctzll(d) >> 3); if (p < jcap) pos = p; }
                    }
                    const unsigned long long bal = xw::ballot(pos != kNone);
                    const uint32_t mine = (uint32_t)(bal >> (i & ~7u)) & 0xFFu;
                    const uint32_t got = xw::shfl(pos, (i & ~7u) + (mine ? (uint32_t)__builtin_ctz(mine) : 0u));
                    if (open && mine) { res = got; open = false; }
                    else if (open && off + 64 >= jcap) { res = jcap; open = false; }
                    off += 64;
                }
                if (have && sub == 0) L->job_len[(jl & 63u) * 4 + (jl >> 8)] = res;
            }
            xw::wave_sync();
#pragma unroll
            for (int k = 0; k < 3; k++) if (cd[k] && cl[k] == kNone) cl[k] = L->job_len[i * 4 + k];
        }

        const unsigned long long f4 = ptick();
        uint32_t *st = L->stage + i * kFtStride;
        uint32_t np = 0, ec = 0, ec_d = kNone, od = kNone, cmpb = 0;
        auto closed_end = [&](uint32_t e, uint32_t d) __attribute__((always_inline)) {
            if (e > ec || (e == ec && d < ec_d)) { ec = e; ec_d = d; }
        };
        auto add_pair = [&](uint32_t d, uint32_t l) __attribute__((always_inline)) {
            if (l >= cap) { od = umin(od, d); return; }
            st[2 + 2 * np] = d; st[3 + 2 * np] = l; np++;
            closed_end(a + l, d);
        };
        if (ht_call) {
            if (cd[0] && 1 < cap) {
                cmpb += cl[0] + (cl[0] < cap);
                if (cl[0] > 1 && cl[0] >= match_min(cd[0])) add_pair(cd[0], cl[0]);
            }
            uint32_t best = 1;
#pragma unroll
            for (int k = 1; k < 3; k++) {
                if (!cd[k] || !(best < cap)) continue;
                cmpb += cl[k] + (cl[k] < cap);
                if (cl[k] > best && cl[k] >= match_min(cd[k])) { add_pair(cd[k], cl[k]); best = cl[k]; }
            }
        }

        uint32_t so_d = 0, so_end = 0;
        auto add_soft = [&](uint32_t d, uint32_t l) __attribute__((always_inline)) {
            st[2 + 2 * np] = d; st[3 + 2 * np] = l; np++;
            if (a + l > so_end || (a + l == so_end && d < so_d)) { so_d = d; so_end = a + l; }
        };
        if (rk_call && rk_act) {
            const uint32_t d = rk_to - rk_from, l = rk_len - (q - rk_to);
            if (l >= match_min(d)) { if (rk_cut && l < cap) add_soft(d, l); else add_pair(d, umin(l, kMatchMax)); }
        }
        uint32_t cut_slot = 64;
        {
            const unsigned long long im = xw::ballot(rk_call && (q & 255u) == 0);
            for (unsigned long long mm = im; mm; mm &= mm - 1) {
                const uint32_t j = (uint32_t)__builtin_ctzll(mm);
                const uint32_t sj = xw::readlane(rkh >> g.rk_shift, j);
                const unsigned long long hit = xw::ballot(rk_probe && i > j && (rkh >> g.rk_shift) == sj);
                if (hit) cut_slot = umin(cut_slot, (uint32_t)__builtin_ctzll(hit));
            }
        }
        if (rk_dropped) cmpb += rk_l16 + 1;
        uint32_t cut_ev = 64, ev_d = 0, ev_l = 0;
        bool ev_ok = false, ev_cut = false;
        {
            const unsigned long long evm = xw::ballot(rk_cand && !rk_dropped);
            if (evm) {
                const uint32_t k = (uint32_t)__builtin_ctzll(evm);
                const uint32_t kd = xw::readlane(rk_d, k), kav = xw::readlane(avail, k) & 0xFFFFu, keff = xw::readlane(rk_eff, k);
                const uint32_t ka = a0 + k;
                const uint32_t l = wave_cmp(G.in, ka - kd, ka, 0, kav);
                cut_ev = k + 1;
                ev_ok = l >= keff && l >= match_min(kd);
                ev_d = kd; ev_l = l;
                ev_cut = l == kav;
                if (i == k) {
                    cmpb += l + (l < kav);
                    if (ev_ok) { if (ev_cut && l < cap) add_soft(kd, l); else add_pair(kd, umin(l, kMatchMax)); }
                }
            }
        }

        const unsigned long long f5 = ptick();
        constexpr uint32_t cut_bin = 64;
        const bool bt_wait = bt_call && i < cut_bin;
        uint32_t bt_n = 0;
        flush_fpos();
        const uint32_t ec0 = ec, ec_d0 = ec_d, od0 = od;
        uint32_t pm = 0, before = 0, js = 64, jo = 64, cut_nice = 64, m = 0;
        bool nice_real = false, so_top = false, so_tie = false, so_win = false;
        unsigned long long stm = 0, om = 0;
        {
            const unsigned long long tw = xw::tick();
            const unsigned long long t0 = xw::clock100();
            uint32_t spins = 0;
            const bool waits = xw::any(bt_wait);
            bool have = !bt_wait;
            uint32_t r_d = 0, r_l = 0;
            bool told = false;
            uint32_t f_seen = 65;
            for (;;) {
                {
                    const unsigned long long ask = xw::ballot(!have);
                    if (ask && i == (uint32_t)__builtin_ctzll(ask)) xw::need_bt(G.hook_user, a);
                }
                if (!have) {
                    const xw::u32x4 q0 = xw::ld_agent128(G.bt_ready + bi * kBtRec);
                    if (q0.x & kBtReady) { have = true; bt_n = q0.x & 0x1FFu; r_d = q0.y; r_l = q0.z; }
                }
                const unsigned long long missing = xw::ballot(!have);
                if (waits && spins == 0) {
                    n_late_unc += (uint32_t)__builtin_popcountll(missing & xw::ballot(unc));
                    n_late_other += (uint32_t)__builtin_popcountll(missing & ~xw::ballot(unc));
                    if (missing) {
                        const bool hot = G.hot_of_bin && !have && G.hot_of_bin[(hash4(v4) >> g.bt_shift) % G.nheads] != 0;
                        n_late_hot += (uint32_t)__builtin_popcountll(xw::ballot(hot));
                        n_late_first += (uint32_t)(missing & 1ull);
                        n_late_blocks++;
                    }
                }
                const uint32_t F = missing ? (uint32_t)__builtin_ctzll(missing) : 64u;
                if (F != f_seen) {
                    f_seen = F;
                    xw::after_poll();
                    ec = ec0; ec_d = ec_d0; od = od0;
                    if (bt_wait && have && bt_n) { if (r_l >= cap) od = umin(od, r_d); else closed_end(a + r_l, r_d); }
                    pm = xw::scan_max(in_blk ? umax(ec, so_end) : 0u);
                    before = umax(xw::lane_below(pm, 0u), reach);
                    if (i >= jc && s_active) before = umax(before, s_end);
                    nice_real = in_blk && umax(before, s_sliding ? s_e : 0u) >= a + kNice;
                    const bool so_free = in_blk && so_end != 0 && od == kNone && !s_sliding;
                    so_tie = so_free && so_end == umax(before, ec);
                    so_win = false;
                    if (xw::any(so_tie)) {
                        uint32_t d2 = kNone;
                        if (ec == so_end) d2 = ec_d;
                        if (reach == so_end) d2 = umin(d2, reach_d);
                        if (i >= jc && s_active && s_end == so_end) d2 = umin(d2, s_d);
                        for (uint32_t j = 0; j + 1 < n; j++) {
                            const uint32_t ej = xw::readlane(ec, j), dj = xw::readlane(ec_d, j), sj = xw::readlane(so_end, j), sdj = xw::readlane(so_d, j);
                            if (j < i && ej == so_end) d2 = umin(d2, dj);
                            if (j < i && sj == so_end) d2 = umin(d2, sdj);
                        }
                        so_win = so_tie && so_d < d2;
                    }
                    so_top = so_free && (so_end > umax(before, ec) || so_win);
                    stm = xw::ballot(so_top);
                    js = stm ? (uint32_t)__builtin_ctzll(stm) : 64u;
                    const unsigned long long bad = xw::ballot(in_blk && nice_real != nice_pred);
                    cut_nice = bad ? (uint32_t)__builtin_ctzll(bad) : 64u;
                    om = xw::ballot(in_blk && od != kNone && (!s_sliding || od < s_d));
                    jo = om ? (uint32_t)__builtin_ctzll(om) : 64u;
                    m = umin(n, umin(cut_nice, umin(jo + 1 > 64 ? 64u : jo + 1, umin(cut_ev, umin(cut_rk, umin(cut_slot, cut_bin))))));
                    m = umin(m, js + 1 > 64 ? 64u : js + 1);
                    if (unc && avail >= 4 && !told && i < umin(F, m)) { xw::st_agent(G.bt_flag + bi, nice_real ? kFlagSkip : kFlagCall); told = true; }
                    if (m <= F) break;
                    if (i == F && unc) xw::st_agent(G.bt_flag + bi, kFlagCall);
                }
                if ((++spins & 63u) == 0) {
                    if (xw::readfirst(xw::ld_agent(&V.hx->err))) { err = kErrInternal + 100; return 1; }
#ifndef NLZM_SIM
                    if (xw::clock100() - t0 > 3000000000ull) {
                        const uint32_t fl = (uint32_t)__builtin_ctzll(missing | (1ull << 63));
                        fail(kErrTimeout, a0 + fl, 6, (uint32_t)__builtin_popcountll(missing) | (xw::readlane(unc ? 1u : 0u, fl) << 8) | (n << 16),
                             xw::readlane((hash4(v4) >> g.bt_shift) % G.nheads, fl));
                        return 1;
                    }
#else
                    (void)t0;
#endif
                }
                xw::pause();
            }
            if (waits) { t_wait += xw::tick() - tw; t_wait_bt += xw::tick() - tw; }
        }

        const unsigned long long f6 = ptick();
        if (m == 0) { fail(kErrInternal, a0, 7); return 1; }
        n_blocks++;
        if (m < n) {
            const uint32_t w = m == cut_nice ? 0u : (m == jo + 1 ? 1u : (m == cut_ev ? 2u : (m == cut_rk ? 3u : (m == cut_bin ? 5u : 4u))));
            n_cut0 += w == 0; n_cut1 += w == 1; n_cut2 += w == 2; n_cut3 += w == 3; n_cut4 += w == 4; n_cut5 += w == 5;
        }
        const bool fin = i < m;
        {
            const unsigned long long gapm = xw::ballot(fin && umax(before, s_sliding ? s_e : 0u) <= a);
            if (gapm) gap_last = a0 + (63u - (uint32_t)__builtin_clzll(gapm));
        }
        if (stm || xw::any(so_tie)) {
            n_so_top += (uint32_t)__builtin_popcountll(xw::ballot(fin && so_top)); n_so_tie += (uint32_t)__builtin_popcountll(xw::ballot(fin && so_tie));
            n_so_won += (uint32_t)__builtin_popcountll(xw::ballot(fin && so_win));
        }

        if (xw::any(fin && nice_real && !unc && avail >= 4 && G.workers)) { fail(kErrV2Promise, a0, 8); return 1; }

        const unsigned long long f7 = ptick();
        for (unsigned long long mm = dep & htm & ((m < 64 ? (1ull << m) : 0ull) - 1ull); mm; mm &= mm - 1) {
            const uint32_t j = (uint32_t)__builtin_ctzll(mm);
            if (i == j) { L->ht2[i2] = e2; L->ht3[i3] = e3; L->ht3[i3 + 1] = r0; }
            xw::wave_sync();
        }
        if (ht_call && i < m && !later) { L->ht2[i2] = e2; L->ht3[i3] = e3; L->ht3[i3 + 1] = r0; }
        xw::wave_sync();
        if (fin && unc && avail >= 4) xw::st_agent(G.bt_flag + bi, nice_real ? kFlagSkip : kFlagCall);
        if (fin && rk_call && (q & 255u) == 0) G.rk_table[rkh >> g.rk_shift] = q | (rkh << g.wbits);
        if (fin) {
            uint32_t w0 = np | (bt_call && bt_n ? kFtBt : 0u) | ((uint32_t)(uint8_t)own0 << 8);
            if (i == jc && s_active && s_end > a + 1) { st[2 + 2 * np] = s_d; st[3 + 2 * np] = s_end - a; np++; w0++; }
            if (s_sliding && i <= jo) { st[14] = s_d; st[15] = cap; w0 |= kFtTop; }
            if (i == jo) { st[14] = od; st[15] = cap; w0 |= kFtTop; }
            st[0] = w0; st[1] = a;
            uint32_t *dst = V.ft + (unsigned long long)(a & (kFtRing - 1)) * kFtStride;
#pragma unroll
            for (int k = 0; k < 4; k++) xw::st_agent128(dst + 4 * k, st[4 * k], st[4 * k + 1], st[4 * k + 2], st[4 * k + 3]);
        }
        {
            const uint32_t last = m - 1;
            const uint32_t pm_last = xw::readlane(pm, last);
            if (pm_last >= reach && pm_last) {
                uint32_t dm = pm_last == reach ? reach_d : kNone;
                const uint32_t le = umax(ec, so_end), ld = umin(ec == le ? ec_d : kNone, so_end == le ? so_d : kNone);
                for (unsigned long long mm = xw::ballot(fin && le == pm_last); mm; mm &= mm - 1) dm = umin(dm, xw::readlane(ld, (uint32_t)__builtin_ctzll(mm)));
                reach = pm_last; reach_d = dm;
            }
            if (s_active && jc <= last) {
                if (s_end > reach) { reach = s_end; reach_d = s_d; } else if (s_end == reach) reach_d = umin(reach_d, s_d);
                s_active = 0;
            }
            if (jo == last) { s_active = 1; s_d = xw::readlane(od, last); s_end = kNone; s_seen = a0 + last + xw::readlane(cap, last); }
            else if (js == last) { s_active = 1; s_d = xw::readlane(so_d, last); s_end = kNone; s_seen = xw::readlane(so_end, last); }
            prev_nice = xw::readlane(nice_real ? 1u : 0u, last);
            const unsigned long long rkf = xw::ballot(fin && rk_call);
            if (rkf) rk_end = (a0 + (63u - (uint32_t)__builtin_clzll(rkf))) - base + 256;
            if (rk_len && xw::any(fin && rk_call && !rk_act)) rk_len = 0;
            if (ev_ok && cut_ev == m) {
                rk_from = (a0 + last - base) - ev_d; rk_to = a0 + last - base; rk_len = ev_l; rk_cut = ev_cut ? 1u : 0u;
            }
        }
        n_pos += m;
        n_nice += (unsigned long long)__builtin_popcountll(xw::ballot(fin && nice_real));
        n_unc += (unsigned long long)__builtin_popcountll(xw::ballot(fin && unc && avail >= 4));
        n_ht += (unsigned long long)__builtin_popcountll(xw::ballot(fin && ht_call));
        n_rkp += (unsigned long long)__builtin_popcountll(xw::ballot(fin && rk_probe));
        n_rki += (unsigned long long)__builtin_popcountll(xw::ballot(fin && rk_call && (q & 255u) == 0));
        n_cmp_lane += fin ? cmpb : 0u;
        pend_fpos = a0 + m;
        pf_a0 = kNone;
        if (a0 + m < a1) {
            pf_a0 = a0 + m;
            const uint32_t na = pf_a0 + i;
            const bool nin = na < a1;
            pf_own0 = nin ? load64u(G.in + na) : 0ull; pf_own1 = nin ? load64u(G.in + na + 8) : 0ull;
            pf_rkh = (nin && la_end - na >= 256) ? G.rkhash[na] : 0u;
            pf_unc = (nin && G.workers) ? G.unc[(unsigned long long)(na - G.batch_a0)] : (uint8_t)0;
        }
        xw::trace(2, a0, n, m, reach, s_active, s_d, s_end);
        {
            const unsigned long long f8 = ptick();
            t_f[0] += f1 - f0; t_f[1] += f2 - f1; t_f[2] += f3 - f2; t_f[3] += f4 - f3; t_f[4] += f5 - f4; t_f[5] += f6 - f5; t_f[6] += f7 - f6; t_f[7] += f8 - f7;
        }
        return m;
    }

    XW_FN void run(uint32_t c0, uint32_t c1)
    {
        FLds *L = xw::lds<FLds>();
        Persist *P = G.persist;
        StateV2 *S = (StateV2 *)V.state;
        const uint32_t i = xw::lane();
        const uint32_t ht3_rows = (1u << (32 - g.ht3_shift)) + 1;
        for (uint32_t k = i; k < 8192; k += 64) L->last[k] = 0;
        for (uint32_t k = i; k < 4096; k += 64) L->ht2[k] = G.ht2[k];
        for (uint32_t k = i; k < ht3_rows; k += 64) L->ht3[k] = G.ht3[k];
        base = xw::readfirst((uint32_t)P->reb_base);
        reach = xw::readfirst(S->reach); reach_d = xw::readfirst(S->reach_d); s_active = xw::readfirst(S->s_active); s_d = xw::readfirst(S->s_d);
        s_end = xw::readfirst(S->s_end); s_seen = xw::readfirst(S->s_seen);
        prev_nice = xw::readfirst(S->prev_nice); seg_s = xw::readfirst(S->seg_s);
        rk_from = xw::readfirst(P->rk_from); rk_to = xw::readfirst(P->rk_to); rk_len = xw::readfirst(P->rk_len); rk_end = xw::readfirst(P->rk_end);
        rk_cut = rk_len >> 31; rk_len &= 0x7FFFFFFFu;
        err = xw::readfirst(P->error);
        if (!err && G.test_fail) fail(kErrInternal + 50, (uint32_t)((unsigned long long)c0 * g.chunk_size), 9);
        n_pos = n_nice = n_unc = n_ht = n_rkp = n_rki = n_cmp = n_blocks = 0;
        n_cut0 = n_cut1 = n_cut2 = n_cut3 = n_cut4 = n_cut5 = 0;
        t_wait = 0;
        const unsigned long long t_start = xw::tick();
        t_pos_seen = (uint32_t)((unsigned long long)c0 * g.chunk_size);
        unsigned long long shifts = 0;
        xw::wave_sync();
        for (uint32_t ci = c0; ci < c1 && !err; ci++) {
            const unsigned long long chunk_abs = (unsigned long long)ci * g.chunk_size;
            const unsigned long long remain = g.n - chunk_abs;
            const uint32_t chunk_read = (uint32_t)(remain < g.feed ? remain : g.feed);
            const uint32_t p_end = umin(g.chunk_size, chunk_read);
            if (chunk_abs - base >= 2ull * (g.wmask + 1)) {
                base += g.wmask + 1;
                shifts++;
                if (i == 0) { L->ht2[0] = kNone; L->ht3[0] = kNone; }
                if (rk_end >= g.wmask + 1) rk_end -= g.wmask + 1; else rk_end = 0;
                xw::wave_sync();
            }
            if (prev_nice) seg_s = (uint32_t)chunk_abs;
            gap_last = (uint32_t)chunk_abs;
            const uint32_t a1 = (uint32_t)chunk_abs + p_end, la_end = (uint32_t)chunk_abs + chunk_read;
            uint32_t a = (uint32_t)chunk_abs;
            while (a < a1 && !err) {
                const uint32_t n = umin(64u, a1 - a);
                dbg_a = a;
                if ((int32_t)(a + n - t_pos_seen - kFtRing) > 0) {
                    flush_fpos();
                    const unsigned long long tw = xw::tick();
                    if (!wait_word_ge(&V.hx->t_pos, a + n - kFtRing, V.hx, 1)) { err = kErrInternal + 100; break; }
                    t_pos_seen = xw::readfirst(xw::ld_agent(&V.hx->t_pos));
                    t_wait += xw::tick() - tw;
                }
                a += block(a, n, a1, la_end);
            }
        }
        flush_fpos();
        for (uint32_t d = 32; d; d >>= 1) n_cmp_lane += xw::shfl64(n_cmp_lane, i ^ d);
        n_cmp += xw::readfirst64(n_cmp_lane);
        xw::wave_sync();
        for (uint32_t k = xw::opaque(i); k < 4096; k += 64) G.ht2[k] = L->ht2[k];
        for (uint32_t k = xw::opaque(i); k < ht3_rows; k += 64) G.ht3[k] = L->ht3[k];
        if (i == 0) {
            P->reb_base = base;
            P->rk_from = rk_from; P->rk_to = rk_to; P->rk_len = rk_len | (rk_cut << 31); P->rk_end = rk_end;
            S->reach = reach; S->reach_d = reach_d; S->s_active = s_active; S->s_d = s_d; S->s_end = s_end; S->s_seen = s_seen;
            S->prev_nice = prev_nice; S->seg_s = seg_s;
            Counters &c = P->cnt;
            xw::atomic_add64_agent(&c.positions, n_pos); xw::atomic_add64_agent(&c.nice_positions, n_nice);
            xw::atomic_add64_agent(&c.uncertain_positions, n_unc); xw::atomic_add64_agent(&c.ht_rows, 3 * n_ht);
            xw::atomic_add64_agent(&c.rk_probes, n_rkp); xw::atomic_add64_agent(&c.rk_inserts, n_rki);
            xw::atomic_add64_agent(&c.cmp_bytes, n_cmp); xw::atomic_add64_agent(&c.shifts, shifts);
            unsigned long long *pr = P->prof;
            xw::atomic_add64_agent(&pr[kPfFinderBlocks], n_blocks); xw::atomic_add64_agent(&pr[kPfFinderCutNice], n_cut0); xw::atomic_add64_agent(&pr[kPfFinderCutTop], n_cut1);
            xw::atomic_add64_agent(&pr[kPfFinderCutRkCand], n_cut2); xw::atomic_add64_agent(&pr[kPfFinderCutRkCatchUp], n_cut3); xw::atomic_add64_agent(&pr[kPfFinderCutOther], n_cut4);
            xw::atomic_add64_agent(&pr[kPfFinderCutBin], n_cut5);
            xw::atomic_add64_agent(&pr[kPfFinderWait], t_wait); xw::atomic_add64_agent(&pr[kPfFinderTotal], xw::tick() - t_start); xw::atomic_add64_agent(&pr[kPfFinderWaitBt], t_wait_bt);
            xw::atomic_add64_agent(&pr[kPfFinderLateUnc], n_late_unc); xw::atomic_add64_agent(&pr[kPfFinderLateOther], n_late_other);
            xw::atomic_add64_agent(&pr[kPfRkShortTop], n_so_top); xw::atomic_add64_agent(&pr[kPfRkShortTie], n_so_tie); xw::atomic_add64_agent(&pr[kPfRkShortWon], n_so_won);
            xw::atomic_add64_agent(&pr[kPfFinderSegOwn], n_seg_own); xw::atomic_add64_agent(&pr[kPfFinderSegWait], n_seg_wait);
            xw::atomic_add64_agent(&pr[kPfFinderLateHot], n_late_hot); xw::atomic_add64_agent(&pr[kPfFinderLateFirst], n_late_first); xw::atomic_add64_agent(&pr[kPfFinderLateBlocks], n_late_blocks);
#ifdef NLZM_PROFILE
            for (uint32_t z = 0; z < kPfFinderSecN; z++) xw::atomic_add64_agent(&pr[kPfFinderSec + z], t_f[z]);
#endif
            if (err || xw::ld_agent(&V.hx->err)) {
                uint32_t *d = V.hx->dbg[kDbgFinder];
                xw::st_agent(&d[kDfBlock], dbg_a); xw::st_agent(&d[kDfReach], reach); xw::st_agent(&d[kDfTopActive], s_active); xw::st_agent(&d[kDfTopDist], s_d);
                xw::st_agent(&d[kDfTopEnd], s_end); xw::st_agent(&d[kDfPrevNice], prev_nice); xw::st_agent(&d[kDfSegStart], seg_s); xw::st_agent(&d[kDfRkLen], rk_len);
                xw::st_agent(&d[kDfTPosSeen], t_pos_seen); xw::st_agent(&d[kDfErr], err); xw::st_agent(&d[kDfBase], base);
            }
        }
    }
};


#ifndef NLZM_FRCAP
#define NLZM_FRCAP 16
#endif
#ifndef NLZM_KTW
#define NLZM_KTW 7
#endif
#ifndef NLZM_FRCAP_WIDE
#define NLZM_FRCAP_WIDE 24
#endif
#ifndef NLZM_KTW_WIDE
#define NLZM_KTW_WIDE 5
#endif
constexpr uint32_t kFrCap = NLZM_FRCAP, kFrCapWide = NLZM_FRCAP_WIDE;
constexpr uint32_t kTW = NLZM_KTW, kTWWide = NLZM_KTW_WIDE;
constexpr uint32_t kTWMax = kTW > kTWWide ? kTW : kTWWide;
constexpr uint32_t kFrArena = (kTW * kFrCap > kTWWide * kFrCapWide ? kTW * kFrCap : kTWWide * kFrCapWide) * 2 * 64;
constexpr uint32_t kTbWidenShift = 6, kTbNarrowShift = 9;
NLZM_HD uint32_t table_waves(uint32_t wide) { return wide ? kTWWide : kTW; }
struct TWave {
    uint32_t recs[64 * kFtStride];
    uint32_t overflow;
};
struct TLds {
    unsigned long long arena[kFrArena];
    TWave w[kTWMax];
    unsigned long long carry[kFrontMax + 8];
    unsigned long long tmp[2 * kFrontMax + 300];
    uint32_t carry_n;
    uint32_t turn;
    uint32_t cursor;
    uint32_t carry_seq;
    uint32_t emit_seq;
    uint32_t stop;
    uint32_t left, sum_blocks, sum_slow;
};

NLZM_HD unsigned long long fr_key(uint32_t e, uint32_t d) { return ((unsigned long long)e << 32) | (0xFFFFFFFFu - d); }
NLZM_HD uint32_t fr_end(unsigned long long k) { return (uint32_t)(k >> 32); }
NLZM_HD uint32_t fr_dist(unsigned long long k) { return 0xFFFFFFFFu - (uint32_t)k; }

struct Table {
    Geom g;
    Globals G;
    GlobalsV2 V;
    uint32_t err;
    uint32_t p_pos_seen;
    uint32_t fcap = kFrCap, nwaves = kTW;
    XW_FN unsigned long long *fronts(uint32_t buf) const { return xw::lds<TLds>()->arena + (unsigned long long)(2 * xw::wave() + buf) * 64 * fcap; }
    unsigned long long n_blocks, n_slow, t_wait;
    unsigned long long n_fr8 = 0, n_fr12 = 0, n_fr16 = 0, n_fr20 = 0, n_fr24 = 0;
    unsigned long long tt0 = 0, tt1 = 0, tt2 = 0, tt3 = 0, tt4 = 0;
#ifdef NLZM_PROFILE
    XW_FN unsigned long long ptick() const { return xw::tick(); }
#else
    XW_FN unsigned long long ptick() const { return 0; }
#endif

    static XW_FN uint32_t merge(const unsigned long long *pa, uint32_t na, const unsigned long long *pb, uint32_t nb, uint32_t low,
                                unsigned long long *out, uint32_t cap)
    {
        while (nb && fr_end(pb[nb - 1]) < low) nb--;
        while (na && fr_end(pa[na - 1]) < low) na--;
        uint32_t ia = 0, ib = 0, no = 0, dmin = kNone;
        unsigned long long ka = na ? pa[0] : 0, kb = nb ? pb[0] : 0;
        while (ia < na || ib < nb) {
            const bool ta = ib >= nb || (ia < na && ka >= kb);
            const unsigned long long k = ta ? ka : kb;
            if (ta) { ia++; ka = ia < na ? pa[ia] : 0; } else { ib++; kb = ib < nb ? pb[ib] : 0; }
            const uint32_t d = fr_dist(k);
            if (d < dmin) {
                if (no >= cap) return kNone;
                out[no++] = k; dmin = d;
            }
        }
        return no;
    }

    XW_FN uint32_t gather(uint32_t a, uint32_t cap_len, const uint32_t *rec, unsigned long long *out, uint32_t cap)
    {
        uint32_t n = 0;
        const uint32_t w0 = rec[0], np = w0 & 7u;
        for (uint32_t k = 0; k < np; k++) {
            if (n >= cap) return kNone;
            out[n++] = fr_key(a + rec[3 + 2 * k], rec[2 + 2 * k]);
        }
        if (w0 & kFtTop) { if (n >= cap) return kNone; out[n++] = fr_key(a + rec[15], rec[14]); }
        if (w0 & kFtBt) {
            const unsigned long long bi = (unsigned long long)(a - G.batch_a0);
            const uint32_t *br = G.bt_ready + bi * kBtRec;
            uint32_t bw[16];
            for (;;) {
#pragma unroll
                for (int k = 0; k < 16; k++) bw[k] = xw::ld_agent(br + k);
                if ((bw[7] & bw[11] & bw[15] & kBtTag) != 0) break;
                if (xw::ld_agent(&V.hx->err)) break;
                xw::pause();
            }
            const uint32_t cnt = bw[0] & 0x1FFu;
#pragma unroll
            for (uint32_t k = 0; k < 4; k++) {
                if (k >= cnt) continue;
                const uint32_t d = bw[bt_rec_d(k)], l = bw[bt_rec_l(k)];
                if (l >= cap_len) continue;
                if (n >= cap) return kNone;
                out[n++] = fr_key(a + l, d);
            }
            const uint32_t *pairs = G.bt_pairs + bi * (2 * G.bt_pstride);
            const bool ext_ok = cnt > G.bt_pstride && bw[14] - 1u < G.bt_ext_cap;
            const uint32_t *extp = ext_ok ? G.bt_ext + (unsigned long long)(bw[14] - 1) * (2 * (kBtMaxPairs - G.bt_pstride)) : pairs;
            const uint32_t cnt_there = (cnt > G.bt_pstride && !ext_ok) ? G.bt_pstride : cnt;
            for (uint32_t k = 4; k < cnt_there; k++) {
                const uint32_t *q = k < G.bt_pstride ? pairs + 2 * k : extp + 2 * (k - G.bt_pstride);
                const uint32_t d = xw::ld_agent(q), l = xw::ld_agent(q + 1);
                if (l >= cap_len) continue;
                if (n >= cap) return kNone;
                out[n++] = fr_key(a + l, d);
            }
        }
        return n;
    }

    static XW_FN uint32_t sort_filter(unsigned long long *v, uint32_t n)
    {
        for (uint32_t x = 1; x < n; x++) {
            const unsigned long long k = v[x];
            uint32_t y = x;
            while (y > 0 && v[y - 1] < k) { v[y] = v[y - 1]; y--; }
            v[y] = k;
        }
        uint32_t no = 0, dmin = kNone;
        for (uint32_t x = 0; x < n; x++) {
            const uint32_t d = fr_dist(v[x]);
            if (d < dmin) { v[no++] = v[x]; dmin = d; }
        }
        return no;
    }

    XW_FN void emit(uint32_t a, uint32_t a1, uint32_t lit, const unsigned long long *f, uint32_t fn)
    {
        uint32_t *rec = V.tp + (unsigned long long)(a & (kTpRing - 1)) * kTpStride;
        uint32_t *fo = V.tf + (unsigned long long)(a & (kTpRing - 1)) * kTfStride;
        const uint32_t mt_max = fn ? fr_end(f[0]) - a : 0u;
        uint32_t max_len = umin(mt_max, a1 - a);
        if (max_len < kMatchMin) max_len = 0;
        uint32_t ne = 0, uniq = 0, dprev = 0;
        if (max_len) {
            uint32_t step = (max_len - kMatchMin) >> 4;
            step += step == 0;
            uint32_t j = 0;
            unsigned long long kj = f[0], kn = fn > 1 ? f[1] : 0;
            unsigned long long held = 0;
            for (uint32_t tl = max_len; tl >= kMatchMin; tl -= umin(tl, step)) {
                while (j + 1 < fn && fr_end(kn) >= a + tl) { j++; kj = kn; kn = j + 1 < fn ? f[j + 1] : 0; }
                const uint32_t d = fr_dist(kj), mm = match_min(d);
                uint32_t nx, ex;
                const uint32_t slot = dist_slot(d - 1, nx, ex);
                const uint32_t valid = tl >= mm ? 1u : 0u, lv = valid ? tl - mm : 0u;
                const uint32_t at = tl | (lv << 9) | (slot << 18) | (nx << 24) | (valid << 31);
                if (ne & 1u) xw::st_agent128(rec + kTpEdges + 2 * (ne - 1), (uint32_t)held, (uint32_t)(held >> 32), d, at);
                else held = (unsigned long long)d | ((unsigned long long)at << 32);
                if (valid && d != dprev) uniq |= 1u << ne;
                if (valid) dprev = d;
                ne++;
            }
            if (ne & 1u) xw::st_agent64((unsigned long long *)(rec + kTpEdges + 2 * (ne - 1)), held);
        }
        xw::st_agent128(rec, ne | (lit << 8) | (mt_max << 16), fn, uniq, 0u);
        for (uint32_t k = 0; k + 1 < fn; k += 2)
            xw::st_agent128(fo + 2 * k, fr_end(f[k]) - a, fr_dist(f[k]), fr_end(f[k + 1]) - a, fr_dist(f[k + 1]));
        if (fn & 1u) xw::st_agent64((unsigned long long *)(fo + 2 * (fn - 1)), (unsigned long long)(fr_end(f[fn - 1]) - a) | ((unsigned long long)fr_dist(f[fn - 1]) << 32));
    }

    XW_FN void capture(uint32_t a, const unsigned long long *f, uint32_t fn);

    XW_FN bool wait_lds(const uint32_t *p, uint32_t v)
    {
        uint32_t spins = 0;
        while (xw::readfirst(xw::lds_ld(p)) != v) {
            if ((++spins & 255u) == 0 && xw::readfirst(xw::ld_agent(&V.hx->err))) return false;
            xw::pause();
        }
        xw::after_poll();
        return true;
    }

    XW_FN void block(uint32_t a0, uint32_t n, uint32_t a1, uint32_t la_end, uint32_t seq)
    {
        TLds *L = xw::lds<TLds>();
        TWave *W = &L->w[xw::wave()];
        const uint32_t i = xw::lane();
        const bool in_blk = i < n;
        const uint32_t a = a0 + i;
        const uint32_t cap_len = in_blk ? umin(la_end - a, kMatchMax) : 0u;
        const uint32_t *rec = V.ft + (unsigned long long)(a & (kFtRing - 1)) * kFtStride;
        uint32_t *r = W->recs + i * kFtStride;
        if (in_blk) {
#pragma unroll
            for (int k = 0; k < 8; k++) {
                const unsigned long long w = xw::ld_agent64((const unsigned long long *)(rec + 2 * k));
                r[2 * k] = (uint32_t)w; r[2 * k + 1] = (uint32_t)(w >> 32);
            }
        } else r[0] = 0;
        const uint32_t lit = (r[0] >> 8) & 0xFFu;
        W->overflow = 0;
        xw::wave_sync();
        const unsigned long long q0 = ptick();
        unsigned long long *mine = fronts(0) + i * fcap;
        uint32_t cnt = 0;
        if (in_blk) {
            cnt = gather(a, cap_len, r, mine, fcap);
            if (cnt == kNone) { W->overflow = 1; cnt = 0; }
            else cnt = sort_filter(mine, cnt);
        }
        const unsigned long long q1 = ptick();
        uint32_t cur = 0, cmax = cnt;
        for (uint32_t D = 1; D < 64; D <<= 1) {
            xw::wave_sync();
            const uint32_t ocnt = xw::shfl_up(cnt, D);
            unsigned long long *dst = fronts(cur ^ 1) + i * fcap;
            const unsigned long long *own = fronts(cur) + i * fcap;
            uint32_t nn;
            if (i >= D && in_blk) nn = merge(own, cnt, fronts(cur) + (i - D) * fcap, ocnt, a + 1, dst, fcap);
            else { for (uint32_t k = 0; k < cnt; k++) dst[k] = own[k]; nn = cnt; }
            if (nn == kNone) { W->overflow = 1; nn = 0; }
            cnt = nn;
            cmax = umax(cmax, cnt);
            cur ^= 1;
        }
        xw::wave_sync();
        const unsigned long long q2 = ptick();
        if (G.cap_words && !wait_lds(&L->emit_seq, seq)) { err = 1; return; }
        if (!wait_lds(&L->carry_seq, seq)) { err = 1; return; }
        const unsigned long long q3 = ptick();
        const uint32_t cn = xw::readfirst(L->carry_n);
        unsigned long long *fin_f = fronts(cur ^ 1) + i * fcap;
        uint32_t fn = 0;
        if (in_blk) {
            fn = merge(fronts(cur) + i * fcap, cnt, L->carry, cn, a + 1, fin_f, fcap);
            if (fn == kNone) { W->overflow = 1; fn = 0; }
        }
        xw::wave_sync();
        n_blocks++;
        cmax = umax(cmax, fn == kNone ? 0u : fn);
        n_fr8 += xw::any(cmax > 8); n_fr12 += xw::any(cmax > 12); n_fr16 += xw::any(cmax > 16); n_fr20 += xw::any(cmax > 20); n_fr24 += xw::any(cmax > 24);
        const bool slow = xw::readfirst(W->overflow) != 0;
        if (slow) slow_block(a0, n, a1, la_end);
        else {
            const uint32_t last_n = xw::readlane(fn, n - 1);
            for (uint32_t k = i; k < last_n; k += 64) L->carry[k] = fronts(cur ^ 1)[(n - 1) * fcap + k];
            if (i == 0) L->carry_n = last_n;
        }
        xw::wave_sync();
        if (i == 0) xw::lds_st(&L->carry_seq, seq + 1);
        const unsigned long long q4 = ptick();
        if (!slow) {
            if (in_blk) emit(a, a1, lit, fin_f, fn);
#ifdef NLZM_SIM
            if (in_blk) sim_on_front(G.hook_user, a, fin_f, fn);
#endif
        }
        xw::drain();
        if (!wait_lds(&L->emit_seq, seq)) { err = 1; return; }
        if (!slow && G.cap_words) {
            for (uint32_t j = 0; j < n; j++) capture(a0 + j, fronts(cur ^ 1) + j * fcap, xw::readlane(fn, j));
        }
        xw::wave_sync();
        if (i == 0) { xw::st_agent(&V.hx->t_out, a0 + n); xw::st_agent(&V.hx->t_pos, a0 + n); xw::lds_st(&L->emit_seq, seq + 1); }
        tt0 += q1 - q0; tt1 += q2 - q1; tt3 += q3 - q2; tt2 += q4 - q3; tt4 += ptick() - q4;
    }

    XW_FN void slow_block(uint32_t a0, uint32_t n, uint32_t a1, uint32_t la_end)
    {
        TLds *L = xw::lds<TLds>();
        TWave *W = &L->w[xw::wave()];
        n_slow++;
        for (uint32_t j = 0; j < n; j++) {
            const uint32_t a = a0 + j;
            const uint32_t cap_len = umin(la_end - a, kMatchMax);
            const uint32_t *rec = V.ft + (unsigned long long)(a & (kFtRing - 1)) * kFtStride;
            uint32_t *r = W->recs;
            if (xw::lane() < 8) {
                const unsigned long long w = xw::ld_agent64((const unsigned long long *)(rec + 2 * xw::lane()));
                r[2 * xw::lane()] = (uint32_t)w; r[2 * xw::lane() + 1] = (uint32_t)(w >> 32);
            }
            xw::wave_sync();
            unsigned long long *t0 = L->tmp, *t1 = L->tmp + 300;
            if (xw::lane() == 0) {
                uint32_t c = gather(a, cap_len, r, t0, 300);
                c = sort_filter(t0, c);
// ... 1290 lines not shown
```

Baseline: 6.645 MB/s.

## Cut scalar register pressure in hot worker and finder roles

The hot worker role now reloads rarely used kernel arguments (bin offsets, ext buffers, abort/progress words, counters) from the kernel argument memory on demand instead of keeping them live in SGPRs. It parks cold scalars in VGPRs and reads them back with readfirstlane, and the extension-buffer fields are only filled when the sink overflows. In the finder, wave-wide ballot/popcount statistics become per-lane counters that are reduced once at the end. The aim is to relieve SGPR pressure and spills in the hot loops, at the cost of extra argument loads and VGPR use on cold paths.

After: 6.875 MB/s (median of 6 runs). +3.5%, better.

```diff
diff --git a/nlzm_amd/csrc/nlzm_kernels.hip b/nlzm_amd/csrc/nlzm_kernels.hip
--- a/nlzm_amd/csrc/nlzm_kernels.hip
+++ b/nlzm_amd/csrc/nlzm_kernels.hip
@@ -377,33 +377,68 @@
     tests_out = tests; cmp_out = cb; n_undo = nu;
 }
 
+#define NLZM_CONST_AS __attribute__((address_space(4)))
+#define NLZM_GLOBAL_AS __attribute__((address_space(1)))
+template <uint32_t kRole, class P> __device__ __forceinline__ P role_args(P p)
+{
+    unsigned long long x = (unsigned long long)p;
+    asm volatile("; the arguments of role %1" : "+s"(x) : "n"(kRole));
+    return (P)x;
+}
+template <bool kFromMemory> __device__ __forceinline__ void global_pointers(Globals &G)
+{
+    if (!kFromMemory) return;
+#define NLZM_GLOBAL_PTR(p) p = (decltype(p))(NLZM_GLOBAL_AS std::remove_pointer_t<decltype(p)> *)(unsigned long long)(p)
+    NLZM_GLOBAL_PTR(G.in); NLZM_GLOBAL_PTR(G.rkhash); NLZM_GLOBAL_PTR(G.ht2); NLZM_GLOBAL_PTR(G.ht3); NLZM_GLOBAL_PTR(G.rk_table);
+    NLZM_GLOBAL_PTR(G.bt_heads); NLZM_GLOBAL_PTR(G.bt_tree); NLZM_GLOBAL_PTR(G.persist); NLZM_GLOBAL_PTR(G.syms); NLZM_GLOBAL_PTR(G.bits);
+    NLZM_GLOBAL_PTR(G.fmeta); NLZM_GLOBAL_PTR(G.cap_words); NLZM_GLOBAL_PTR(G.cap_used); NLZM_GLOBAL_PTR(G.bt_ready); NLZM_GLOBAL_PTR(G.bt_pairs); NLZM_GLOBAL_PTR(G.bt_ext); NLZM_GLOBAL_PTR(G.bt_ext_cur);
+    NLZM_GLOBAL_PTR(G.bt_flag); NLZM_GLOBAL_PTR(G.unc); NLZM_GLOBAL_PTR(G.bin_off); NLZM_GLOBAL_PTR(G.bin_pos); NLZM_GLOBAL_PTR(G.abort_word);
+    NLZM_GLOBAL_PTR(G.progress); NLZM_GLOBAL_PTR(G.wcnt); NLZM_GLOBAL_PTR(G.bt_undo); NLZM_GLOBAL_PTR(G.hot_of_bin); NLZM_GLOBAL_PTR(G.hot_list); NLZM_GLOBAL_PTR(G.hot_undo);
+}
+template <bool kFromMemory, class T> __device__ __forceinline__ T *global_pointer(T *p)
+{
+    return kFromMemory ? (T *)(NLZM_GLOBAL_AS T *)(unsigned long long)p : p;
+}
+template <bool kFromMemory> __device__ __forceinline__ void global_pointers(v2::GlobalsV2 &V)
+{
+    if (!kFromMemory) return;
+    NLZM_GLOBAL_PTR(V.ft); NLZM_GLOBAL_PTR(V.tp); NLZM_GLOBAL_PTR(V.tf); NLZM_GLOBAL_PTR(V.hx); NLZM_GLOBAL_PTR(V.state); NLZM_GLOBAL_PTR(V.hb);
+#undef NLZM_GLOBAL_PTR
+}
+__device__ __forceinline__ uint32_t parked(uint32_t v) { asm volatile("" : "+v"(v)); return v; }
+__device__ __forceinline__ unsigned long long parked(unsigned long long v) { asm volatile("" : "+v"(v)); return v; }
+__device__ __forceinline__ uint32_t unparked(uint32_t v) { return (uint32_t)__builtin_amdgcn_readfirstlane((int)v); }
+__device__ __forceinline__ unsigned long long unparked(unsigned long long v) { return ((unsigned long long)unparked((uint32_t)(v >> 32)) << 32) | unparked((uint32_t)v); }
 #ifndef NLZM_RISKY_AHEAD
 #define NLZM_RISKY_AHEAD 0
 #endif
 constexpr uint32_t kPending = 0xFFFFFFFEu;
 __device__ __forceinline__ uint32_t wave_max_u32(uint32_t v) { return (uint32_t)__builtin_amdgcn_readlane((int)xw::scan_max(v), 63); }
-__device__ __forceinline__ void worker_role_hot(const Geom &g, const Globals &G, uint32_t c0, uint32_t c1, uint32_t bin, uint32_t hot_index)
+template <bool kFromMemory, class P>
+__device__ __forceinline__ void worker_role_hot(P args, const Geom &g, const Globals &G, uint32_t c0, uint32_t c1, uint32_t bin, uint32_t hot_index)
 {
     unsigned long long p0 = (unsigned long long)G.in, p1 = (unsigned long long)G.bt_heads, p2 = (unsigned long long)G.bt_tree,
                        p3 = (unsigned long long)G.bt_ready, p4 = (unsigned long long)G.bt_pairs, p5 = (unsigned long long)G.bt_flag,
                        p6 = (unsigned long long)G.hot_undo;
     uint32_t q0 = G.batch_a0, q2 = g.wmask, q3 = g.bt_tmask;
-    asm volatile("" : "+s"(p0), "+s"(p1), "+s"(p2), "+s"(p3), "+s"(p4), "+s"(p5), "+s"(p6));
+    asm volatile("" : "+s"(p0), "+s"(p1), "+s"(p2), "+s"(p5), "+s"(p6));
+    p3 = parked(p3); p4 = parked(p4);
     asm volatile("" : "+s"(q0), "+s"(q2), "+s"(q3));
 #define NLZM_AS_GLOBAL(T, x) ((T *)(__attribute__((address_space(1))) T *)(x))
     const uint8_t *in = NLZM_AS_GLOBAL(const uint8_t, p0);
-    uint32_t *heads = NLZM_AS_GLOBAL(uint32_t, p1), *tree = NLZM_AS_GLOBAL(uint32_t, p2), *ready = NLZM_AS_GLOBAL(uint32_t, p3);
-    uint32_t *pairs = NLZM_AS_GLOBAL(uint32_t, p4);
+    uint32_t *heads = NLZM_AS_GLOBAL(uint32_t, p1), *tree = NLZM_AS_GLOBAL(uint32_t, p2);
+#define NLZM_HOT_READY NLZM_AS_GLOBAL(uint32_t, unparked(p3))
+#define NLZM_HOT_PAIRS NLZM_AS_GLOBAL(uint32_t, unparked(p4))
     const uint32_t *flags = NLZM_AS_GLOBAL(const uint32_t, p5);
     const uint32_t lane = threadIdx.x & 63u;
     unsigned long long *const undo = NLZM_AS_GLOBAL(unsigned long long, p6) + ((unsigned long long)hot_index * 64 + lane) * kUndoCap;
-#undef NLZM_AS_GLOBAL
     const uint32_t batch_a0 = q0, wmask = q2, tmask = q3;
-    BtView Bx{ in, heads, tree, ready, pairs, batch_a0, 0u, wmask, tmask };
-    Bx.pstride = G.bt_pstride; Bx.ext = G.bt_ext; Bx.ext_cur = G.bt_ext_cur; Bx.ext_cap = G.bt_ext_cap; Bx.fail_word = G.abort_word;
+    BtView Bx{ in, heads, tree, nullptr, nullptr, batch_a0, 0u, wmask, tmask };
+    Bx.pstride = G.bt_pstride;
     enum : uint32_t { kIdle = 0, kStart = 1, kRun = 2, kHeld = 3 };
     enum : uint32_t { kwNone = 0, kwDone = 1, kwPark = 2, kwCall = 3 };
-    uint32_t c = c0, wb = 0, cur = 0, e0 = 0, la_end = 0;
+    uint32_t c = parked(c0), wb = 0, cur = 0, e0 = 0, la_end = 0;
+    const uint32_t c0p = parked(c0), c1p = parked(c1), binp = parked(bin);
     const uint32_t *pos = G.bin_pos;
     bool loaded = false, more = true, wvalid = false, rec = false;
     unsigned long long w_pe = 0;
@@ -420,13 +455,14 @@
     LaneSink sink{ (uint32_t *)&g_v2_lds + threadIdx.x, nullptr };
     unsigned long long n_tests = 0, n_cmp = 0;
     uint32_t n_calls = 0, n_open = 0, n_back = 0, n_redo = 0;
-    uint32_t n_steps = 0, n_blk_risky = 0;
-    unsigned long long t_wait0 = 0;
-    uint32_t prog_seen = 0, steps = 0;
+    uint32_t n_steps = parked(0u), n_blk_risky = parked(0u);
+    unsigned long long t_wait0 = parked(0ull);
+    uint32_t prog_seen = parked(0u), steps = 0;
     uint32_t k_work = 0, k_tests = 0, k_rep = 0, k_rec = 0, k_full = 0, k_blk = 0, k_noent = 0, k_skip = 0, k_und = 0;
-    const unsigned long long k_t0 = __builtin_readcyclecounter();
+    const unsigned long long k_t0 = parked((unsigned long long)__builtin_readcyclecounter());
     uint32_t k_total = 0;
     for (uint32_t cc = c0; cc < c1; cc++) { const uint32_t *off = G.bin_off + (unsigned long long)(cc - c0) * (G.nheads + 1); k_total += off[bin + 1] - off[bin]; }
+    k_total = parked(k_total);
 #ifdef NLZM_PROFILE
     unsigned long long t_sec[7] = {}, t_last = __builtin_readcyclecounter();
 #define NLZM_HOT_STAMP(k) do { const unsigned long long t_now = __builtin_readcyclecounter(); t_sec[k] += t_now - t_last; t_last = t_now; } while (0)
@@ -443,18 +479,21 @@
         if (!wvalid && more && !rec) {
             for (;;) {
                 if (!loaded) {
-                    if (c >= c1) { more = false; break; }
-                    const uint32_t *off = G.bin_off + (unsigned long long)(c - c0) * (G.nheads + 1);
-                    cur = (uint32_t)__builtin_amdgcn_readfirstlane((int)off[bin]); e0 = (uint32_t)__builtin_amdgcn_readfirstlane((int)off[bin + 1]);
-                    const unsigned long long chunk_abs = (unsigned long long)c * g.chunk_size;
-                    const unsigned long long remain = g.n - chunk_abs;
-                    la_end = (uint32_t)(chunk_abs + (remain < g.feed ? remain : g.feed));
-                    pos = G.bin_pos + (unsigned long long)(c - c0) * g.chunk_size * 2;
+                    const uint32_t cu = unparked(c), cfirst = unparked(c0p), bin_u = unparked(binp);
+                    if (cu >= unparked(c1p)) { more = false; break; }
+                    const P A = role_args<10>(args);
+                    const uint32_t *off = global_pointer<kFromMemory>(A->G.bin_off) + (unsigned long long)(cu - cfirst) * (A->G.nheads + 1);
+                    cur = (uint32_t)__builtin_amdgcn_readfirstlane((int)off[bin_u]); e0 = (uint32_t)__builtin_amdgcn_readfirstlane((int)off[bin_u + 1]);
+                    const uint32_t chunk_size = A->g.chunk_size, feed = A->g.feed;
+                    const unsigned long long chunk_abs = (unsigned long long)cu * chunk_size;
+                    const unsigned long long remain = A->g.n - chunk_abs;
+                    la_end = (uint32_t)(chunk_abs + (remain < feed ? remain : feed));
+                    pos = global_pointer<kFromMemory>(A->G.bin_pos) + (unsigned long long)(cu - cfirst) * chunk_size * 2;
                     loaded = true;
                 }
                 if (cur < e0) break;
                 if (__any(st != kIdle) || ovalid) break;
-                c++; loaded = false;
+                c = parked(unparked(c) + 1); loaded = false;
             }
             if (more && loaded && cur < e0) {
                 wb = cur;
@@ -630,7 +669,7 @@
                 started_now = true;
                 sp = v_word;
                 pend_l = (a & tmask) << 1; pend_r = pend_l + 1; len_l = 0; len_r = 0; tests = 0; cb = 0; cmp_off = 0;
-                sink.count = 0; sink.best = 1; sink.best_d = 0; sink.ext_idx = 0; sink.pairs = pairs + (unsigned long long)(a - batch_a0) * (2 * Bx.pstride);
+                sink.count = 0; sink.best = 1; sink.best_d = 0; sink.ext_idx = 0; sink.pairs = NLZM_HOT_PAIRS + (unsigned long long)(a - batch_a0) * (2 * Bx.pstride);
                 published = false;
                 undo[0] = (0x80000000u | hidx) | ((unsigned long long)sp << 32);
                 nu = 1;
@@ -659,7 +698,16 @@
                 tests++;
                 cb += (l - init) + (full ? 0u : 1u);
                 const uint32_t d = a - sp;
-                if (l >= match_min(d) && l > sink.best) sink.put(Bx, d, l);
+                if (l >= match_min(d) && l > sink.best) {
+                    if (sink.count < 4) sink.put(Bx, d, l);
+                    else {
+                        const P A = role_args<13>(args);
+                        BtView Be = Bx;
+                        Be.ext = global_pointer<kFromMemory>(A->G.bt_ext); Be.ext_cur = global_pointer<kFromMemory>(A->G.bt_ext_cur); Be.ext_cap = A->G.bt_ext_cap;
+                        Be.fail_word = global_pointer<kFromMemory>(A->G.abort_word);
+                        sink.put(Be, d, l);
+                    }
+                }
                 if (full) { fin_now = true; fin_l = pl; fin_r = pr; }
                 else {
                     const uint32_t slot = right ? pend_l : pend_r;
@@ -681,7 +729,7 @@
             st = kHeld;
         }
         if (st == kHeld && !wrong) {
-            if (!published && seq <= oseq) { sink.publish(ready + (unsigned long long)(a - batch_a0) * kBtRec, tests); published = true; }
+            if (!published && seq <= oseq) { sink.publish(NLZM_HOT_READY + (unsigned long long)(a - batch_a0) * kBtRec, tests); published = true; }
             if (published && !und && seq <= oseq) {
                 n_calls++; n_tests += tests; n_cmp += cb;
                 st = kIdle;
@@ -705,20 +753,24 @@
         (void)made_test; (void)rep_step; (void)started_now;
 #endif
         if ((++steps & 4095u) == 0) {
-            if (__any(LaneIO::ld_agent(G.abort_word) != 0)) break;
+            const P A = role_args<11>(args);
+            uint32_t *const abort_word = global_pointer<kFromMemory>(A->G.abort_word);
+            const uint32_t *const progress = global_pointer<kFromMemory>(A->G.progress);
+            if (__any(LaneIO::ld_agent(abort_word) != 0)) break;
             if (__any(und || w_und || o_und)) {
                 const unsigned long long now = wall_clock64();
-                const uint32_t prog = G.progress ? (uint32_t)__builtin_amdgcn_readfirstlane((int)LaneIO::ld_agent(G.progress)) : 0u;
-                if (!t_wait0 || prog != prog_seen) { t_wait0 = now; prog_seen = prog; }
-                else if (now - t_wait0 > 3000000000ull) { if (lane == 0) LaneIO::st_agent(G.abort_word, 2u); break; }
-            } else t_wait0 = 0;
+                const uint32_t prog = progress ? (uint32_t)__builtin_amdgcn_readfirstlane((int)LaneIO::ld_agent(progress)) : 0u;
+                if (!unparked(t_wait0) || prog != unparked(prog_seen)) { t_wait0 = parked(now); prog_seen = parked(prog); }
+                else if (now - unparked(t_wait0) > 3000000000ull) { if (lane == 0) LaneIO::st_agent(abort_word, 2u); break; }
+            } else t_wait0 = parked(0ull);
         }
         NLZM_HOT_STAMP(5);
         if (!more && !wvalid && !ovalid && !rec && !__any(st != kIdle)) break;
     }
+    WorkerCounters *const wcnt = global_pointer<kFromMemory>(role_args<12>(args)->G.wcnt);
     if (st != kIdle) {
-        atomicAdd(&G.wcnt->stuck_lanes, 1ull);
-        atomicMax(&G.wcnt->stuck_pos_inv, (unsigned long long)(uint32_t)~a);
+        atomicAdd(&wcnt->stuck_lanes, 1ull);
+        atomicMax(&wcnt->stuck_pos_inv, (unsigned long long)(uint32_t)~a);
     }
     unsigned long long t_calls = n_calls, t_open = n_open, t_back = n_back, t_redo = n_redo, t_skip = k_skip;
     for (int m = 32; m >= 1; m >>= 1) {
@@ -727,24 +779,29 @@
         t_skip += __shfl_xor(t_skip, m, 64);
     }
     if (lane == 0) {
-        atomicAdd(&G.wcnt->bt_calls, t_calls); atomicAdd(&G.wcnt->bt_tests, n_tests); atomicAdd(&G.wcnt->cmp_bytes, n_cmp);
-        atomicAdd(&G.wcnt->dry_runs, t_open); atomicAdd(&G.wcnt->spec_calls, t_back); atomicAdd(&G.wcnt->spec_good, t_redo);
-        atomicAdd(&G.wcnt->hot_calls, t_calls);
-        atomicAdd(&G.wcnt->hot_steps, (unsigned long long)n_steps); atomicAdd(&G.wcnt->hot_blocked_risky, (unsigned long long)n_blk_risky);
+        atomicAdd(&wcnt->bt_calls, t_calls); atomicAdd(&wcnt->bt_tests, n_tests); atomicAdd(&wcnt->cmp_bytes, n_cmp);
+        atomicAdd(&wcnt->dry_runs, t_open); atomicAdd(&wcnt->spec_calls, t_back); atomicAdd(&wcnt->spec_good, t_redo);
+        atomicAdd(&wcnt->hot_calls, t_calls);
+        atomicAdd(&wcnt->hot_steps, (unsigned long long)unparked(n_steps)); atomicAdd(&wcnt->hot_blocked_risky, (unsigned long long)unparked(n_blk_risky));
         uint32_t kc = 0;
-        while (kc < 7 && (k_total >> (14 + kc))) kc++;
-        unsigned long long *hc = G.wcnt->hot_class[kc];
-        atomicAdd(&hc[kHcWaves], 1ull); atomicAdd(&hc[kHcCalls], t_calls); atomicAdd(&hc[kHcTests], n_tests); atomicAdd(&hc[kHcSteps], (unsigned long long)n_steps); atomicAdd(&hc[kHcTestSteps], (unsigned long long)k_work);
+        const uint32_t k_all = unparked(k_total);
+        while (kc < 7 && (k_all >> (14 + kc))) kc++;
+        unsigned long long *hc = wcnt->hot_class[kc];
+        atomicAdd(&hc[kHcWaves], 1ull); atomicAdd(&hc[kHcCalls], t_calls); atomicAdd(&hc[kHcTests], n_tests); atomicAdd(&hc[kHcSteps], (unsigned long long)unparked(n_steps)); atomicAdd(&hc[kHcTestSteps], (unsigned long long)k_work);
         atomicAdd(&hc[kHcLaneTests], (unsigned long long)k_tests); atomicAdd(&hc[kHcRepeats], (unsigned long long)k_rep); atomicAdd(&hc[kHcTakingBack], (unsigned long long)k_rec); atomicAdd(&hc[kHcAllHold], (unsigned long long)k_full); atomicAdd(&hc[kHcMayNotStart], (unsigned long long)k_blk);
-        atomicAdd(&hc[kHcNoEntry], (unsigned long long)k_noent); atomicAdd(&hc[kHcCycles], (unsigned long long)(__builtin_readcyclecounter() - k_t0)); atomicAdd(&hc[kHcSkipped], t_skip); atomicAdd(&hc[kHcIdleUndecided], (unsigned long long)k_und);
+        atomicAdd(&hc[kHcNoEntry], (unsigned long long)k_noent); atomicAdd(&hc[kHcCycles], (unsigned long long)(__builtin_readcyclecounter() - unparked(k_t0))); atomicAdd(&hc[kHcSkipped], t_skip); atomicAdd(&hc[kHcIdleUndecided], (unsigned long long)k_und);
 #ifdef NLZM_PROFILE
         for (uint32_t z = 0; z < kHcSecN; z++) atomicAdd(&hc[kHcSec + z], t_sec[z]);
 #endif
     }
 #undef NLZM_HOT_STAMP
-}
-
-__device__ __forceinline__ void worker_role(const Geom &g, const Globals &G, uint32_t c0, uint32_t c1, uint32_t wblocks, uint32_t wblock)
+#undef NLZM_HOT_READY
+#undef NLZM_HOT_PAIRS
+#undef NLZM_AS_GLOBAL
+}
+
+template <bool kFromMemory, class P>
+__device__ __forceinline__ void worker_role(P args, const Geom &g, const Globals &G, uint32_t c0, uint32_t c1, uint32_t wblocks, uint32_t wblock)
 {
     constexpr uint32_t kLpw = NLZM_LPW;
     const uint32_t lane_waves = (G.wthreads + kLpw - 1) / kLpw;
@@ -752,7 +809,7 @@
         if (!G.hot_list) return;
         const uint32_t k = ((threadIdx.x >> 6) - lane_waves) * wblocks + wblock;
         if (k >= G.hot_list[0]) return;
-        worker_role_hot(g, G, c0, c1, G.hot_list[1 + k], k);
+        worker_role_hot<kFromMemory>(args, g, G, c0, c1, G.hot_list[1 + k], k);
         return;
     }
     const uint32_t lane_in_block = (threadIdx.x >> 6) * kLpw + (threadIdx.x & 63u);
@@ -915,17 +972,44 @@
 }
 
 constexpr uint32_t kV2Roles = 3 + v2::kHelpers;
-__device__ __forceinline__ void pipeline2_roles(const Geom &g, const Globals &G, const v2::GlobalsV2 &V, uint32_t c0, uint32_t c1,
-                                                uint32_t local_block, uint32_t wblocks)
+struct Pipe2Args { Geom g; Globals G; v2::GlobalsV2 V; uint32_t c0, c1; };
+struct Stream2Args { Geom g; Globals G; v2::GlobalsV2 V; uint32_t c0, c1; v2::RoundSnap *snap; };
+static_assert(offsetof(Stream2Args, g) == offsetof(Pipe2Args, g) && offsetof(Stream2Args, G) == offsetof(Pipe2Args, G) && offsetof(Stream2Args, V) == offsetof(Pipe2Args, V) &&
+              offsetof(Stream2Args, c0) == offsetof(Pipe2Args, c0) && offsetof(Stream2Args, c1) == offsetof(Pipe2Args, c1), "a Stream2Args starts with a Pipe2Args");
+template <bool kFromMemory, class R, class P> __device__ __forceinline__ void stage_args(R &r, P a)
+{
+    __builtin_memcpy(&r.g, &a->g, sizeof(Geom)); __builtin_memcpy(&r.G, &a->G, sizeof(Globals)); __builtin_memcpy(&r.V, &a->V, sizeof(v2::GlobalsV2));
+    global_pointers<kFromMemory>(r.G); global_pointers<kFromMemory>(r.V);
+}
+template <bool kFromMemory, class P> __device__ __forceinline__ void pipeline2_roles(P args, uint32_t local_block, uint32_t wblocks)
 {
     if (local_block < kV2Roles) {
-        if (threadIdx.x >= (local_block >= 2 ? v2::kParserThreads : (local_block == 1 ? 64u * v2::table_waves(((const v2::StateV2 *)V.state)->tb_wide[G.launch_par & 1u]) : 64u))) return;
-        if (local_block == 0) { v2::Finder r; r.g = g; r.G = G; r.V = V; r.run(c0, c1); }
-        else if (local_block == 1) { v2::Table r; r.g = g; r.G = G; r.V = V; r.run(c0, c1); }
-        else if (local_block == 2) { v2::Parser r; r.g = g; r.G = G; r.V = V; r.run(c0, c1); }
-        else if (V.hb) { v2::Parser r; r.g = g; r.G = G; r.V = V; r.run_helper(c0, local_block - 3); }
+        if (local_block == 0) {
+            if (threadIdx.x >= 64u) return;
+            const P a = role_args<0>(args);
+            v2::Finder r; stage_args<kFromMemory>(r, a); r.run(a->c0, a->c1);
+        } else if (local_block == 1) {
+            const P a = role_args<1>(args);
+            v2::Table r; stage_args<kFromMemory>(r, a);
+            if (threadIdx.x >= 64u * v2::table_waves(((const v2::StateV2 *)r.V.state)->tb_wide[r.G.launch_par & 1u])) return;
+            r.run(a->c0, a->c1);
+        } else {
+            if (threadIdx.x >= v2::kParserThreads) return;
+            if (local_block == 2) {
+                const P a = role_args<2>(args);
+                v2::Parser r; stage_args<kFromMemory>(r, a); r.run(a->c0, a->c1);
+            } else {
+                const P a = role_args<3>(args);
+                v2::Parser r; stage_args<kFromMemory>(r, a);
+                if (r.V.hb) r.run_helper(a->c0, local_block - 3);
+            }
+        }
     } else {
-        worker_role(g, G, c0, c1, wblocks, local_block - kV2Roles);
+        const P a = role_args<4>(args);
+        Geom g; Globals G;
+        __builtin_memcpy(&g, &a->g, sizeof(Geom)); __builtin_memcpy(&G, &a->G, sizeof(Globals));
+        global_pointers<kFromMemory>(G);
+        worker_role<kFromMemory>(a, g, G, a->c0, a->c1, wblocks, local_block - kV2Roles);
     }
 }
 __global__ __launch_bounds__(512) void pipeline2_kernel(Geom g, Globals G, v2::GlobalsV2 V, uint32_t c0, uint32_t c1)
@@ -934,24 +1018,15 @@
     const bool spread = gridDim.x > 8 * (kV2Roles - 1);
     const uint32_t before = b ? (b + 7) / 8 < kV2Roles ? (b + 7) / 8 : kV2Roles : 0u;
     const uint32_t local = (b % 8 == 0 && b / 8 < kV2Roles && spread) ? b / 8 : (spread ? kV2Roles + (b - before) : b);
-    pipeline2_roles(g, G, V, c0, c1, local, gridDim.x - kV2Roles);
-}
-struct Stream2Args { Geom g; Globals G; v2::GlobalsV2 V; uint32_t c0, c1; v2::RoundSnap *snap; };
+    (void)g; (void)G; (void)V; (void)c0; (void)c1;
+    pipeline2_roles<false>((const NLZM_CONST_AS Pipe2Args *)__builtin_amdgcn_kernarg_segment_ptr(), local, gridDim.x - kV2Roles);
+}
 constexpr uint32_t kMaxStreams2PerLaunch = 64;
 __global__ __launch_bounds__(512) void pipeline2_multi_kernel(const Stream2Args *__restrict__ pack, uint32_t bps)
 {
     uint32_t s, local;
     multi_block_of(gridDim.x, bps, blockIdx.x, s, local);
-    Stream2Args a = pack[s];
-#define NLZM_GLOBAL_PTR(p) p = (decltype(p))(__attribute__((address_space(1))) std::remove_pointer_t<decltype(p)> *)(unsigned long long)(p)
-    NLZM_GLOBAL_PTR(a.G.in); NLZM_GLOBAL_PTR(a.G.rkhash); NLZM_GLOBAL_PTR(a.G.ht2); NLZM_GLOBAL_PTR(a.G.ht3); NLZM_GLOBAL_PTR(a.G.rk_table);
-    NLZM_GLOBAL_PTR(a.G.bt_heads); NLZM_GLOBAL_PTR(a.G.bt_tree); NLZM_GLOBAL_PTR(a.G.persist); NLZM_GLOBAL_PTR(a.G.syms); NLZM_GLOBAL_PTR(a.G.bits);
-    NLZM_GLOBAL_PTR(a.G.fmeta); NLZM_GLOBAL_PTR(a.G.cap_words); NLZM_GLOBAL_PTR(a.G.cap_used); NLZM_GLOBAL_PTR(a.G.bt_ready); NLZM_GLOBAL_PTR(a.G.bt_pairs); NLZM_GLOBAL_PTR(a.G.bt_ext); NLZM_GLOBAL_PTR(a.G.bt_ext_cur);
-    NLZM_GLOBAL_PTR(a.G.bt_flag); NLZM_GLOBAL_PTR(a.G.unc); NLZM_GLOBAL_PTR(a.G.bin_off); NLZM_GLOBAL_PTR(a.G.bin_pos); NLZM_GLOBAL_PTR(a.G.abort_word);
-    NLZM_GLOBAL_PTR(a.G.progress); NLZM_GLOBAL_PTR(a.G.wcnt); NLZM_GLOBAL_PTR(a.G.bt_undo); NLZM_GLOBAL_PTR(a.G.hot_of_bin); NLZM_GLOBAL_PTR(a.G.hot_list); NLZM_GLOBAL_PTR(a.G.hot_undo);
-    NLZM_GLOBAL_PTR(a.V.ft); NLZM_GLOBAL_PTR(a.V.tp); NLZM_GLOBAL_PTR(a.V.tf); NLZM_GLOBAL_PTR(a.V.hx); NLZM_GLOBAL_PTR(a.V.state); NLZM_GLOBAL_PTR(a.V.hb);
-#undef NLZM_GLOBAL_PTR
-    pipeline2_roles(a.g, a.G, a.V, a.c0, a.c1, local, bps - kV2Roles);
+    pipeline2_roles<true>((const NLZM_CONST_AS Stream2Args *)(unsigned long long)(pack + s), local, bps - kV2Roles);
 }
 #define NLZM_G(T, x) ((__attribute__((address_space(1))) T *)(unsigned long long)(x))
 __global__ __launch_bounds__(256) void round_open_kernel(const Stream2Args *__restrict__ pack)
diff --git a/nlzm_amd/csrc/nlzm_v2.h b/nlzm_amd/csrc/nlzm_v2.h
--- a/nlzm_amd/csrc/nlzm_v2.h
+++ b/nlzm_amd/csrc/nlzm_v2.h
@@ -156,15 +156,24 @@
     uint32_t rk_cut = 0;
     uint32_t prev_nice, seg_s;
     uint32_t gap_last = 0;
-    uint32_t n_seg_own = 0, n_seg_wait = 0;
     uint32_t t_pos_seen;
     uint32_t err;
     uint32_t dbg_a = 0;
-    unsigned long long n_pos, n_nice, n_unc, n_ht, n_rkp, n_rki, n_cmp, n_blocks, n_cut0, n_cut1, n_cut2, n_cut3, n_cut4, n_cut5;
+    uint32_t n_pos = 0, n_nice = 0, n_unc = 0, n_ht = 0, n_rkp = 0, n_rki = 0;
     unsigned long long n_cmp_lane = 0;
     unsigned long long t_wait, t_wait_bt = 0, t_total;
     uint32_t n_so_top = 0, n_so_tie = 0, n_so_won = 0;
-    uint32_t n_late_unc = 0, n_late_other = 0, n_late_hot = 0, n_late_first = 0, n_late_blocks = 0;
+    uint32_t n_late_unc = 0, n_late_other = 0, n_late_hot = 0;
+    enum : uint32_t { kWcCut0 = 0, kWcBlocks = 6, kWcLateFirst = 7, kWcLateBlocks = 8, kWcSegOwn = 9, kWcSegWait = 10 };
+    uint32_t n_wave = 0;
+    XW_FN void count(uint32_t k, uint32_t v = 1) { n_wave += xw::lane() == k ? v : 0u; }
+    XW_FN unsigned long long counted(uint32_t k) const { return xw::readlane(n_wave, k); }
+    XW_FN unsigned long long lane_sum(uint32_t v) const
+    {
+        unsigned long long t = v;
+        for (uint32_t d = 32; d; d >>= 1) t += xw::shfl64(t, xw::lane() ^ d);
+        return xw::readfirst64(t);
+    }
     unsigned long long t_f[kPfFinderSecN] = {};
 #ifdef NLZM_PROFILE
     XW_FN unsigned long long ptick() const { return xw::tick(); }
@@ -236,7 +245,7 @@
                     if (covered || own) {
                         xw::after_poll();
                         seg_s = sa;
-                        n_seg_own += own; n_seg_wait += spins != 0;
+                        count(kWcSegOwn, own); count(kWcSegWait, spins != 0);
                         xw::trace(1, a0, seg_s, (uint32_t)ps);
                         break;
                     }
@@ -266,7 +275,7 @@
                 for (uint32_t e = (rk_end | 255u) + 1; e < q0 + 256; e += 256) {
                     const uint32_t hh = xw::readfirst(G.rkhash[base + e - 256]);
                     if (i == 0) G.rk_table[hh >> g.rk_shift] = q0 | (hh << g.wbits);
-                    n_rki++;
+                    n_rki += i == 0;
                 }
                 xw::drain();
             }
@@ -505,13 +514,12 @@
                 }
                 const unsigned long long missing = xw::ballot(!have);
                 if (waits && spins == 0) {
-                    n_late_unc += (uint32_t)__builtin_popcountll(missing & xw::ballot(unc));
-                    n_late_other += (uint32_t)__builtin_popcountll(missing & ~xw::ballot(unc));
+                    n_late_unc += !have && unc;
+                    n_late_other += !have && !unc;
                     if (missing) {
                         const bool hot = G.hot_of_bin && !have && G.hot_of_bin[(hash4(v4) >> g.bt_shift) % G.nheads] != 0;
-                        n_late_hot += (uint32_t)__builtin_popcountll(xw::ballot(hot));
-                        n_late_first += (uint32_t)(missing & 1ull);
-                        n_late_blocks++;
+                        n_late_hot += hot;
+                        count(kWcLateFirst, (uint32_t)(missing & 1ull)); count(kWcLateBlocks);
                     }
                 }
                 const uint32_t F = missing ? (uint32_t)__builtin_ctzll(missing) : 64u;
@@ -572,10 +580,10 @@
 
         const unsigned long long f6 = ptick();
         if (m == 0) { fail(kErrInternal, a0, 7); return 1; }
-        n_blocks++;
+        count(kWcBlocks);
         if (m < n) {
             const uint32_t w = m == cut_nice ? 0u : (m == jo + 1 ? 1u : (m == cut_ev ? 2u : (m == cut_rk ? 3u : (m == cut_bin ? 5u : 4u))));
-            n_cut0 += w == 0; n_cut1 += w == 1; n_cut2 += w == 2; n_cut3 += w == 3; n_cut4 += w == 4; n_cut5 += w == 5;
+            count(kWcCut0 + w);
         }
         const bool fin = i < m;
         {
@@ -583,8 +591,7 @@
             if (gapm) gap_last = a0 + (63u - (uint32_t)__builtin_clzll(gapm));
         }
         if (stm || xw::any(so_tie)) {
-            n_so_top += (uint32_t)__builtin_popcountll(xw::ballot(fin && so_top)); n_so_tie += (uint32_t)__builtin_popcountll(xw::ballot(fin && so_tie));
-            n_so_won += (uint32_t)__builtin_popcountll(xw::ballot(fin && so_win));
+            n_so_top += fin && so_top; n_so_tie += fin && so_tie; n_so_won += fin && so_win;
         }
 
         if (xw::any(fin && nice_real && !unc && avail >= 4 && G.workers)) { fail(kErrV2Promise, a0, 8); return 1; }
@@ -632,12 +639,12 @@
                 rk_from = (a0 + last - base) - ev_d; rk_to = a0 + last - base; rk_len = ev_l; rk_cut = ev_cut ? 1u : 0u;
             }
         }
-        n_pos += m;
-        n_nice += (unsigned long long)__builtin_popcountll(xw::ballot(fin && nice_real));
-        n_unc += (unsigned long long)__builtin_popcountll(xw::ballot(fin && unc && avail >= 4));
-        n_ht += (unsigned long long)__builtin_popcountll(xw::ballot(fin && ht_call));
-        n_rkp += (unsigned long long)__builtin_popcountll(xw::ballot(fin && rk_probe));
-        n_rki += (unsigned long long)__builtin_popcountll(xw::ballot(fin && rk_call && (q & 255u) == 0));
+        n_pos += fin;
+        n_nice += fin && nice_real;
+        n_unc += fin && unc && avail >= 4;
+        n_ht += fin && ht_call;
+        n_rkp += fin && rk_probe;
+        n_rki += fin && rk_call && (q & 255u) == 0;
         n_cmp_lane += fin ? cmpb : 0u;
         pend_fpos = a0 + m;
         pf_a0 = kNone;
@@ -675,8 +682,6 @@
         rk_cut = rk_len >> 31; rk_len &= 0x7FFFFFFFu;
         err = xw::readfirst(P->error);
         if (!err && G.test_fail) fail(kErrInternal + 50, (uint32_t)((unsigned long long)c0 * g.chunk_size), 9);
-        n_pos = n_nice = n_unc = n_ht = n_rkp = n_rki = n_cmp = n_blocks = 0;
-        n_cut0 = n_cut1 = n_cut2 = n_cut3 = n_cut4 = n_cut5 = 0;
         t_wait = 0;
         const unsigned long long t_start = xw::tick();
         t_pos_seen = (uint32_t)((unsigned long long)c0 * g.chunk_size);
@@ -713,7 +718,13 @@
         }
         flush_fpos();
         for (uint32_t d = 32; d; d >>= 1) n_cmp_lane += xw::shfl64(n_cmp_lane, i ^ d);
-        n_cmp += xw::readfirst64(n_cmp_lane);
+        const unsigned long long s_cmp = xw::readfirst64(n_cmp_lane);
+        const unsigned long long s_pos = lane_sum(n_pos), s_nice = lane_sum(n_nice), s_unc = lane_sum(n_unc), s_ht = lane_sum(n_ht), s_rkp = lane_sum(n_rkp), s_rki = lane_sum(n_rki);
+        const unsigned long long s_so_top = lane_sum(n_so_top), s_so_tie = lane_sum(n_so_tie), s_so_won = lane_sum(n_so_won);
+        const unsigned long long s_late_unc = lane_sum(n_late_unc), s_late_other = lane_sum(n_late_other), s_late_hot = lane_sum(n_late_hot);
+        const unsigned long long s_blocks = counted(kWcBlocks), s_cut0 = counted(kWcCut0), s_cut1 = counted(kWcCut0 + 1), s_cut2 = counted(kWcCut0 + 2), s_cut3 = counted(kWcCut0 + 3),
+                                 s_cut4 = counted(kWcCut0 + 4), s_cut5 = counted(kWcCut0 + 5), s_late_first = counted(kWcLateFirst), s_late_blocks = counted(kWcLateBlocks),
+                                 s_seg_own = counted(kWcSegOwn), s_seg_wait = counted(kWcSegWait);
         xw::wave_sync();
         for (uint32_t k = xw::opaque(i); k < 4096; k += 64) G.ht2[k] = L->ht2[k];
         for (uint32_t k = xw::opaque(i); k < ht3_rows; k += 64) G.ht3[k] = L->ht3[k];
@@ -723,19 +734,19 @@
             S->reach = reach; S->reach_d = reach_d; S->s_active = s_active; S->s_d = s_d; S->s_end = s_end; S->s_seen = s_seen;
             S->prev_nice = prev_nice; S->seg_s = seg_s;
             Counters &c = P->cnt;
-            xw::atomic_add64_agent(&c.positions, n_pos); xw::atomic_add64_agent(&c.nice_positions, n_nice);
-            xw::atomic_add64_agent(&c.uncertain_positions, n_unc); xw::atomic_add64_agent(&c.ht_rows, 3 * n_ht);
-            xw::atomic_add64_agent(&c.rk_probes, n_rkp); xw::atomic_add64_agent(&c.rk_inserts, n_rki);
-            xw::atomic_add64_agent(&c.cmp_bytes, n_cmp); xw::atomic_add64_agent(&c.shifts, shifts);
+            xw::atomic_add64_agent(&c.positions, s_pos); xw::atomic_add64_agent(&c.nice_positions, s_nice);
+            xw::atomic_add64_agent(&c.uncertain_positions, s_unc); xw::atomic_add64_agent(&c.ht_rows, 3 * s_ht);
+            xw::atomic_add64_agent(&c.rk_probes, s_rkp); xw::atomic_add64_agent(&c.rk_inserts, s_rki);
+            xw::atomic_add64_agent(&c.cmp_bytes, s_cmp); xw::atomic_add64_agent(&c.shifts, shifts);
             unsigned long long *pr = P->prof;
-            xw::atomic_add64_agent(&pr[kPfFinderBlocks], n_blocks); xw::atomic_add64_agent(&pr[kPfFinderCutNice], n_cut0); xw::atomic_add64_agent(&pr[kPfFinderCutTop], n_cut1);
-            xw::atomic_add64_agent(&pr[kPfFinderCutRkCand], n_cut2); xw::atomic_add64_agent(&pr[kPfFinderCutRkCatchUp], n_cut3); xw::atomic_add64_agent(&pr[kPfFinderCutOther], n_cut4);
-            xw::atomic_add64_agent(&pr[kPfFinderCutBin], n_cut5);
+            xw::atomic_add64_agent(&pr[kPfFinderBlocks], s_blocks); xw::atomic_add64_agent(&pr[kPfFinderCutNice], s_cut0); xw::atomic_add64_agent(&pr[kPfFinderCutTop], s_cut1);
+            xw::atomic_add64_agent(&pr[kPfFinderCutRkCand], s_cut2); xw::atomic_add64_agent(&pr[kPfFinderCutRkCatchUp], s_cut3); xw::atomic_add64_agent(&pr[kPfFinderCutOther], s_cut4);
+            xw::atomic_add64_agent(&pr[kPfFinderCutBin], s_cut5);
             xw::atomic_add64_agent(&pr[kPfFinderWait], t_wait); xw::atomic_add64_agent(&pr[kPfFinderTotal], xw::tick() - t_start); xw::atomic_add64_agent(&pr[kPfFinderWaitBt], t_wait_bt);
-            xw::atomic_add64_agent(&pr[kPfFinderLateUnc], n_late_unc); xw::atomic_add64_agent(&pr[kPfFinderLateOther], n_late_other);
-            xw::atomic_add64_agent(&pr[kPfRkShortTop], n_so_top); xw::atomic_add64_agent(&pr[kPfRkShortTie], n_so_tie); xw::atomic_add64_agent(&pr[kPfRkShortWon], n_so_won);
-            xw::atomic_add64_agent(&pr[kPfFinderSegOwn], n_seg_own); xw::atomic_add64_agent(&pr[kPfFinderSegWait], n_seg_wait);
-            xw::atomic_add64_agent(&pr[kPfFinderLateHot], n_late_hot); xw::atomic_add64_agent(&pr[kPfFinderLateFirst], n_late_first); xw::atomic_add64_agent(&pr[kPfFinderLateBlocks], n_late_blocks);
+            xw::atomic_add64_agent(&pr[kPfFinderLateUnc], s_late_unc); xw::atomic_add64_agent(&pr[kPfFinderLateOther], s_late_other);
+            xw::atomic_add64_agent(&pr[kPfRkShortTop], s_so_top); xw::atomic_add64_agent(&pr[kPfRkShortTie], s_so_tie); xw::atomic_add64_agent(&pr[kPfRkShortWon], s_so_won);
+            xw::atomic_add64_agent(&pr[kPfFinderSegOwn], s_seg_own); xw::atomic_add64_agent(&pr[kPfFinderSegWait], s_seg_wait);
+            xw::atomic_add64_agent(&pr[kPfFinderLateHot], s_late_hot); xw::atomic_add64_agent(&pr[kPfFinderLateFirst], s_late_first); xw::atomic_add64_agent(&pr[kPfFinderLateBlocks], s_late_blocks);
 #ifdef NLZM_PROFILE
             for (uint32_t z = 0; z < kPfFinderSecN; z++) xw::atomic_add64_agent(&pr[kPfFinderSec + z], t_f[z]);
 #endif
```
